# FanmingL/Recurrent-Offpolicy-RL

Hardware: AMD Instinct MI355X
Metric: env-steps/sec trained (higher is better)
Workload: dtype f32; 1 GPU; smamba_s32_c16_b2_nln SAC-REDQ update, B=64/GPU, T=1024, D=256 (configs[1]; N=8: configs[3]); row_length=1043, obs=17, act=6, critic=efc-8, global_rows=64, parallelism=dp1

## Files before the change

include/resel_hip.h:

```cpp
#ifndef RESEL_HIP_H
#define RESEL_HIP_H

#include <stddef.h>
#include <stdint.h>

#ifdef __cplusplus
extern "C" {
#endif

#define RESEL_OK 0
#define RESEL_EINVAL (-1)
#define RESEL_ELAUNCH (-2)

typedef void* resel_stream_t;

int resel_abi_version(void);
const char* resel_build_info(void);

enum {
    RESEL_PROF_SSCAN_FWD = 0, RESEL_PROF_SSCAN_BWD = 1, RESEL_PROF_ATTN_FWD = 2, RESEL_PROF_ATTN_DQ = 3, RESEL_PROF_ATTN_DKV = 4,
    RESEL_PROF_LINREC_REAL_FWD = 5, RESEL_PROF_LINREC_REAL_BWD = 6, RESEL_PROF_LINREC_COMPLEX_FWD = 7, RESEL_PROF_LINREC_COMPLEX_BWD = 8,
    RESEL_PROF_GRU_FWD = 9, RESEL_PROF_GRU_BWD = 10, RESEL_PROF_CONV_FWD = 11, RESEL_PROF_CONV_BWD = 12, RESEL_PROF_GEMM = 13,
    RESEL_PROF_SSCAN_FWD_LOCAL = 14, RESEL_PROF_SSCAN_BWD_LOCAL = 15,
    RESEL_PROF_NSLOTS = 16
};
int resel_profile_enable(int on);
int resel_profile_collect(int kernel_id, double* total_us, int* launches);

#define RESEL_SSCAN_CKPT 8
size_t resel_selective_scan_ckpt_bytes(int B, int L, int Di, int N);
size_t resel_selective_scan_fwd_workspace_bytes(int B, int L, int Di, int N, int time_segments);
int resel_selective_scan_fwd(const float* u, int64_t ld_u, const float* delta, int64_t ld_delta,
                             const float* z, int64_t ld_z, const float* A,
                             const float* Bm, int64_t ld_b, const float* Cm, int64_t ld_c,
                             const float* D, const float* delta_bias, const float* start,
                             float* out, int64_t ld_out, float* ckpt, float* last_state, void* workspace,
                             int B, int L, int Di, int N, int delta_softplus, int time_segments,
                             void* amax_out, unsigned amax_epoch, resel_stream_t stream);

size_t resel_selective_scan_bwd_workspace_bytes(int B, int L, int Di, int N, int time_segments);
int resel_selective_scan_bwd(const float* u, int64_t ld_u, const float* delta, int64_t ld_delta,
                             const float* z, int64_t ld_z, const float* A,
                             const float* Bm, int64_t ld_b, const float* Cm, int64_t ld_c,
                             const float* D, const float* delta_bias, const float* start,
                             const float* dout, int64_t ld_dout, const float* ckpt,
                             float* du, int64_t ld_du, float* ddelta, int64_t ld_ddelta, float* dz, int64_t ld_dz,
                             float* dBm, int64_t ld_db, float* dCm, int64_t ld_dc,
                             float* dA, float* dD, float* ddelta_bias, void* workspace,
                             int B, int L, int Di, int N, int delta_softplus, int time_segments,
                             void* amax_dz, void* amax_ddelta, unsigned amax_epoch, resel_stream_t stream);

int resel_causal_conv1d_fwd(const float* x, int64_t ld_x, const float* w, const float* bias, const float* mask,
                            float* y, int64_t ld_y, int B, int L, int Di, int K, int silu, void* amax_y, unsigned amax_epoch,
                            resel_stream_t stream);
size_t resel_causal_conv1d_bwd_workspace_bytes(int B, int L, int Di, int K);
int resel_causal_conv1d_bwd(const float* x, int64_t ld_x, const float* w, const float* bias, const float* mask,
                            const float* dy, int64_t ld_dy, float* dx, int64_t ld_dx, float* dw, float* dbias,
                            void* workspace, int B, int L, int Di, int K, int silu, void* amax_dx, unsigned amax_epoch,
                            resel_stream_t stream);
int resel_causal_conv1d_bwd2(const float* x, int64_t ld_x, const float* w, const float* bias, const float* mask,
                             const float* dy, int64_t ld_dy, const float* dy2, int64_t ld_dy2, float* dx, int64_t ld_dx,
                             float* dw, float* dbias, void* workspace, int B, int L, int Di, int K, int silu,
                             void* amax_dx, unsigned amax_epoch, resel_stream_t stream);

int resel_add_layernorm_fwd(const float* x, const float* residual, const float* w, const float* b,
                            float* y, float* res_out, float* stats, int M, int C, float eps, int rms, int act,
                            void* amax_y, unsigned amax_epoch, resel_stream_t stream);
size_t resel_add_layernorm_bwd_workspace_bytes(int M, int C);
int resel_add_layernorm_bwd(const float* dy, const float* dres_in, const float* res, const float* w, const float* b,
                            const float* stats, float* dx, float* dw, float* db, void* workspace,
                            int M, int C, int rms, int has_bias, int act, void* amax_dx, unsigned amax_epoch, resel_stream_t stream);

int resel_linrec_real_fwd(const float* v, const float* f, int64_t ld_u, const float* start, const float* h0, float* h,
                          int B, int L, int C, int fuse_act, void* amax_h, unsigned amax_epoch, resel_stream_t stream);
int resel_linrec_real_bwd(const float* v, const float* f, int64_t ld_u, const float* start, const float* h0, const float* h,
                          const float* dh, float* dv, float* df, int64_t ld_du, int B, int L, int C, int fuse_act,
                          void* amax_du, unsigned amax_epoch, resel_stream_t stream);
int resel_linrec_complex_fwd(const float* vr, const float* vi, int64_t ld_u, const float* lam_re, const float* lam_im,
                             const float* gamma, const float* start, const float* h0r, const float* h0i,
                             float* hr, float* hi, int B, int L, int C, void* amax_h, unsigned amax_epoch, resel_stream_t stream);
size_t resel_linrec_complex_bwd_workspace_bytes(int B, int L, int C);
int resel_linrec_complex_bwd(const float* vr, const float* vi, int64_t ld_u, const float* lam_re, const float* lam_im,
                             const float* gamma, const float* start, const float* h0r, const float* h0i,
                             const float* hr, const float* hi, const float* dhr, const float* dhi,
                             float* dvr, float* dvi, int64_t ld_du, float* dlam_re, float* dlam_im, float* dgamma,
                             void* workspace, int B, int L, int C, resel_stream_t stream);

int resel_lru_params_fwd(const float* params_log, float* out, int C, resel_stream_t stream);
int resel_lru_params_bwd(const float* params_log, const float* dout, float* dparams_log, int C, resel_stream_t stream);

size_t resel_gru_workspace_bytes(int B, int L, int H);
int resel_gru_seq_fwd(const float* gi, const float* w_hh, const float* b_hh, const float* h0,
                      float* h_all, float* gates, void* workspace, int B, int L, int H, resel_stream_t stream);
int resel_gru_seq_bwd(const float* w_hh, const float* h0, const float* h_all, const float* gates,
                      const float* dh_all, float* dgi, float* dgh, void* workspace,
                      int B, int L, int H, resel_stream_t stream);

size_t resel_gru_multi_workspace_bytes(int n_net, int B, int L, int H);
int resel_gru_multi_fwd(int n_net, const float* const* gi, const float* const* w_hh, const float* const* b_hh,
                        const float* const* h0, float* const* h_all, float* const* gates, void* workspace,
                        int B, int L, int H, resel_stream_t stream);
int resel_gru_multi_form(int n_net, int B, int H);

size_t resel_attn_varlen_fwd_workspace_bytes(int S, int max_seqlen);
int resel_attn_varlen_fwd(const uint16_t* qkv, const int32_t* cu_seqlens, const float* slopes, uint16_t* out, float* lse,
                          void* workspace, int T, int S, int H, int hd, int max_seqlen, float scale,
                          float p_drop, uint64_t seed, uint64_t offset, resel_stream_t stream);
size_t resel_attn_varlen_bwd_workspace_bytes(int T, int S, int H, int hd, int max_seqlen);
int resel_attn_varlen_bwd(const uint16_t* qkv, const int32_t* cu_seqlens, const float* slopes, const uint16_t* out,
                          const float* lse, const uint16_t* dout, uint16_t* dqkv, void* workspace,
                          int T, int S, int H, int hd, int max_seqlen, float scale,
                          float p_drop, uint64_t seed, uint64_t offset, resel_stream_t stream);

int resel_dropout(const float* x, float* y, int64_t n, float p_drop, uint64_t seed, uint64_t offset, resel_stream_t stream);
int resel_dropout_offset_base(const void* base);
int resel_gelu_dropout_fwd(const float* x, float* y, int64_t n, float p_drop, uint64_t seed, uint64_t offset,
                           void* amax_y, unsigned amax_epoch, resel_stream_t stream);
int resel_gelu_dropout_bwd(const float* x, const float* dy, float* dx, int64_t n, float p_drop, uint64_t seed, uint64_t offset,
                           void* amax_dx, unsigned amax_epoch, resel_stream_t stream);

int resel_tanh_gaussian_fwd(const float* out2, const float* noise, float* action_mean, float* action_sample,
                            float* logp, int M, int A, resel_stream_t stream);
int resel_tanh_gaussian_bwd(const float* out2, const float* noise, const float* d_sample, const float* d_logp,
                            float* d_out2, int M, int A, resel_stream_t stream);

int resel_sac_target(const float* q, const int32_t* subset, int m, const float* next_logp, const float* log_alpha,
                     const float* reward, const float* done, const float* mask, float gamma, float* guard,
                     float* target, float* stats, void* workspace, int E, int M, resel_stream_t stream);
int resel_sac_target_phase(int phase, const float* q, const int32_t* subset, int m, const float* next_logp, const float* log_alpha,
                           const float* reward, const float* done, const float* mask, float gamma, float* guard,
                           float* target, float* stats, float* extrema, void* workspace, int E, int M, resel_stream_t stream);
int resel_sac_target_local(const float* q, const int32_t* subset, int m, const float* next_logp, const float* log_alpha,
                           const float* reward, const float* done, const float* mask, float gamma, const float* guard,
                           float* target, float* stats, float* extrema, void* workspace, int E, int M, resel_stream_t stream);
int resel_guard_apply_slots(const float* slots, int world, float* guard, resel_stream_t stream);
size_t resel_sac_target_workspace_bytes(int M);

size_t resel_masked_loss_workspace_bytes(void);
int resel_q_loss_fwd(const float* q, const float* y, const float* mask, float* out2, void* workspace, int E, int M, resel_stream_t stream);
int resel_q_loss_bwd(const float* q, const float* y, const float* mask, const float* g, float* dq, int E, int M, resel_stream_t stream);
int resel_actor_loss_fwd(const float* logp, const float* q, const float* mask, const float* log_alpha, float* out2, void* workspace,
                         int E, int M, int use_logp, int reduce_min, resel_stream_t stream);
int resel_actor_loss_bwd(const float* q, const float* mask, const float* log_alpha, const float* g, float* dlogp, float* dq,
                         int E, int M, int use_logp, int reduce_min, resel_stream_t stream);

int resel_soft_update(float* target, const float* online, float tau, int64_t n, resel_stream_t stream);
int resel_adamw_flat(float* p, const float* g, float* m, float* v, int64_t n, const int64_t* seg_end,
                     const float* seg_lr, const float* seg_wd, int nseg, float beta1, float beta2, float eps,
                     int step, const float* grad_scale, resel_stream_t stream);
int resel_adamw_flat_bc(float* p, const float* g, float* m, float* v, int64_t n, const int64_t* seg_end,
                        const float* seg_lr, const float* seg_wd, int nseg, float beta1, float beta2, float eps,
                        float bc1, float bc2_sqrt, const float* grad_scale, resel_stream_t stream);
int resel_adamw_flat_dev(float* p, const float* g, float* m, float* v, int64_t n, const int64_t* seg_end,
                         const float* seg_lr, const float* seg_wd, int nseg, float beta1, float beta2, float eps,
                         const float* bias_corrections, const float* grad_scale, resel_stream_t stream);
size_t resel_sumsq_workspace_bytes(int64_t n);
int resel_sumsq(const float* x, int64_t n, float* out, void* workspace, resel_stream_t stream);

int resel_bias_act_fwd(float* y, const float* bias, int64_t rows, int C, int64_t rows_per_seg, int act, resel_stream_t stream);
size_t resel_bias_act_bwd_workspace_bytes(int64_t rows, int C, int64_t rows_per_seg);
int resel_bias_act_bwd(const float* g, int64_t ldg, const float* a, int64_t lda, float* gy, float* dbias, void* workspace, int64_t rows, int C,
                       int64_t rows_per_seg, int act, void* amax_gy, unsigned amax_epoch, resel_stream_t stream);

int resel_ensemble_head_fwd(float* y, const float* b2, const float* w3, const float* b3, float* q, int64_t rows, int H,
                            int64_t rows_per_seg, resel_stream_t stream);
size_t resel_ensemble_head_bwd_workspace_bytes(int64_t rows, int H, int64_t rows_per_seg);
int resel_ensemble_head_bwd(const float* gq, const float* a, const float* w3, float* gy, float* db2, float* dw3, void* workspace,
                            int64_t rows, int H, int64_t rows_per_seg, void* amax_gy, unsigned amax_epoch, resel_stream_t stream);

size_t resel_gemm_f32_workspace_bytes(int M, int N, int K, int batch);
int resel_gemm_f32(const float* A, int64_t lda, int64_t strideA, int a_kcontig,
                   const float* B, int64_t ldb, int64_t strideB, int b_kcontig,
                   const float* bias, int64_t strideBias, int act,
                   float* C, int64_t ldc, int64_t strideC, void* workspace,
                   int M, int N, int K, int batch, int split, resel_stream_t stream);

int resel_gemm_f32x(const float* A, int64_t lda, int64_t strideA, int a_kcontig,
                    const float* B, int64_t ldb, int64_t strideB, int b_kcontig,
                    const float* bias, int64_t strideBias, int act,
                    float* C, int64_t ldc, int64_t strideC, void* workspace,
                    int M, int N, int K, int batch, int split, const float* amax_a, const float* amax_b,
                    void* amax_c, unsigned amax_epoch, resel_stream_t stream);
int resel_gemm_f32_fused_supported(int kind, int M, int N, int K, int64_t lda, int64_t ldb);
size_t resel_gemm_f32_fused_workspace_bytes(int M, int N, int K, int batch, int kind);
int resel_gemm_f32_dact(const float* A, int64_t lda, int64_t strideA, int a_kcontig,
                        const float* B, int64_t ldb, int64_t strideB, int b_kcontig,
                        const float* Y, int64_t ldy, int64_t strideY,
                        float* C, int64_t ldc, int64_t strideC, float* dbias, void* workspace,
                        int M, int N, int K, int batch, const float* amax_a, const float* amax_b,
                        void* amax_c, unsigned amax_epoch, resel_stream_t stream);
int resel_gemm_f32_head(const float* A, int64_t lda, int64_t strideA, int a_kcontig,
                        const float* B, int64_t ldb, int64_t strideB, int b_kcontig,
                        const float* bias, int64_t strideBias, const float* w3, int64_t strideW3, const float* b3,
                        float* C, int64_t ldc, int64_t strideC, float* q, void* workspace,
                        int M, int N, int K, int batch, const float* amax_a, const float* amax_b,
                        void* amax_c, unsigned amax_epoch, resel_stream_t stream);
int resel_place_blocks(float* out, int64_t ld_out, int rows, int cols, int nblk, const float* const* src, const int64_t* ld_src,
                       const int* r0, const int* nr, const int* c0, const int* nc, resel_stream_t stream);

int resel_amax_segments(const float* flat, const int64_t* begin, const int64_t* len, int nseg, void* handles, unsigned epoch,
                        resel_stream_t stream);
size_t resel_amax_state_bytes(void);
int resel_amax(const float* x, int64_t ld, int64_t stride, int rows, int cols, int batch, void* out, unsigned epoch, void* state,
               resel_stream_t stream);
int resel_amax_check(const float* x, int64_t ld, int64_t stride, int rows, int cols, int batch, const void* handle, int* err, int tag,
                     resel_stream_t stream);

size_t resel_gemm_bf16_workspace_bytes(int M, int N, int K);
int resel_gemm_bf16(const void* A, int64_t lda, int a_kcontig, int a_bf16, const void* B, int64_t ldb, int b_kcontig, int b_bf16,
                    const float* bias, void* C, int64_t ldc, int c_bf16, void* workspace, int M, int N, int K,
                    resel_stream_t stream);

size_t resel_colsum_bf16_workspace_bytes(int M, int N);
int resel_colsum_bf16(const uint16_t* x, int64_t ld, int M, int N, float* out, void* workspace, resel_stream_t stream);

int resel_gather_trajs(const float* buffer, int W, int64_t capacity, const int* segments, int nseg, int max_len, int skip, int rows, int Tp,
                       int c_mask, int c_start, int c_done, int c_timeout, const int* pre_pairs, int npairs,
                       float* out, resel_stream_t stream);

int resel_mamba_conv_step(const float* x, int64_t ldx, const float* state_in, int64_t ld_in, float* state_out, int64_t ld_out,
                          int64_t stride_d, int64_t stride_k, int W, const float* w, const float* bias, float* xc, int B, int Di,
                          int K, int act, resel_stream_t stream);
int resel_selective_state_update(const float* state_in, int64_t ld_in, float* state_out, int64_t ld_out, const float* xc,
                                 const float* x_db, int64_t ld_xdb, const float* w_dt, const float* dt_bias, const float* A_log,
                                 const float* D, const float* z, int64_t ldz, float* y, int B, int Di, int N, int R,
                                 resel_stream_t stream);
int resel_attn_decode(const uint16_t* qkv, int64_t ld_qkv, uint16_t* kv_cache, const int32_t* pos_dev, int pos_host,
                      const float* slopes, uint16_t* out, float scale, int B, int H, int head_dim, int max_seqlen,
                      resel_stream_t stream);

size_t resel_atb_workspace_bytes(int64_t K, int Wd, int Nd);
int resel_atb(const float* wide, int64_t ldw, int Wd, const float* narrow, int64_t ldn, int Nd, float* out, int transposed,
              void* workspace, int64_t K, resel_stream_t stream);

#ifdef __cplusplus
}
#endif
#endif
```

recurrent-offpolicy-rl_amd/csrc/gemm_bf3.hip:

```cpp
#include "gemm_splitk.h"
#include <type_traits>

namespace {
using namespace resel;

typedef float f32x16 __attribute__((ext_vector_type(16)));
typedef __bf16 bf16x8 __attribute__((ext_vector_type(8)));
constexpr int BM = 256, BN = 128;
constexpr int NTH = 512;
constexpr int GRID = 256;
constexpr int TILE = BM * BN;
constexpr int ROWB = 64;
constexpr int PLA = BM * ROWB, PLB = BN * ROWB;
constexpr int STAGE = 3 * PLA + 3 * PLB;

struct Params {
    const float *A, *B, *bias;
    float *C, *slab;
    int64_t lda, ldb, ldc, sA, sB, sC, sBias;
    int M, N, K;
    int act;
    int mt, nt;
    int nfull, nsplit, nsl, kslice;
    const float *amaxA, *amaxB;
    AmaxOut amaxC;
    int ntst;
    const float* aux;
    int64_t ldaux, sAux;
    float* red;
    int redrows;
};

__device__ __forceinline__ int plane_off(int row, int c) {
    const int q = row >> 2;
    return ((row ^ (q & 1)) << 6) + ((c ^ (q & 3)) << 4);
}

__device__ __forceinline__ uint32_t rne_pair(float lo, float hi) {
    typedef __bf16 bf16x2_t __attribute__((ext_vector_type(2)));
    typedef float f32x2_t __attribute__((ext_vector_type(2)));
    const f32x2_t v = {lo, hi};
    return __builtin_bit_cast(uint32_t, __builtin_convertvector(v, bf16x2_t));
}
struct P3 { uint2 p1, p2, p3; };
template <int NP>
__device__ __forceinline__ P3 split4(const float4& v) {
#ifdef BF3_AB_NOSPLIT
    return P3{make_uint2(__float_as_uint(v.x), __float_as_uint(v.y)), make_uint2(__float_as_uint(v.z), __float_as_uint(v.w)),
              make_uint2(__float_as_uint(v.x), __float_as_uint(v.w))};
#endif
    const float x[4] = {v.x, v.y, v.z, v.w};
    uint32_t w1[2], w2[2], w3[2] = {0u, 0u};
#pragma unroll
    for (int q = 0; q < 2; ++q) {
        const uint32_t u0 = __float_as_uint(x[2 * q]), u1 = __float_as_uint(x[2 * q + 1]);
        w1[q] = __builtin_amdgcn_perm(u1, u0, 0x07060302u);
        const float r0 = x[2 * q] - __uint_as_float(u0 & 0xffff0000u), r1 = x[2 * q + 1] - __uint_as_float(u1 & 0xffff0000u);
        if (NP == 2) {
            w2[q] = rne_pair(r0, r1);
        } else {
            const uint32_t v0 = __float_as_uint(r0), v1 = __float_as_uint(r1);
            w2[q] = __builtin_amdgcn_perm(v1, v0, 0x07060302u);
            const float s0 = r0 - __uint_as_float(v0 & 0xffff0000u), s1 = r1 - __uint_as_float(v1 & 0xffff0000u);
            w3[q] = __builtin_amdgcn_perm(__float_as_uint(s1), __float_as_uint(s0), 0x07060302u);
        }
    }
    return P3{make_uint2(w1[0], w1[1]), make_uint2(w2[0], w2[1]), make_uint2(w3[0], w3[1])};
}
struct P3h { uint32_t p1, p2, p3; };
template <int NP>
__device__ __forceinline__ P3h split2(float x0, float x1) {
    const uint32_t u0 = __float_as_uint(x0), u1 = __float_as_uint(x1);
    P3h o;
    o.p1 = __builtin_amdgcn_perm(u1, u0, 0x07060302u);
    const float r0 = x0 - __uint_as_float(u0 & 0xffff0000u), r1 = x1 - __uint_as_float(u1 & 0xffff0000u);
    if (NP == 2) {
        o.p2 = rne_pair(r0, r1);
        o.p3 = 0u;
        return o;
    }
    const uint32_t v0 = __float_as_uint(r0), v1 = __float_as_uint(r1);
    o.p2 = __builtin_amdgcn_perm(v1, v0, 0x07060302u);
    const float s0 = r0 - __uint_as_float(v0 & 0xffff0000u), s1 = r1 - __uint_as_float(v1 & 0xffff0000u);
    o.p3 = __builtin_amdgcn_perm(__float_as_uint(s1), __float_as_uint(s0), 0x07060302u);
    return o;
}

typedef _Float16 f16x2_t __attribute__((ext_vector_type(2)));
typedef float f32x2_t __attribute__((ext_vector_type(2)));
template <bool WIDE>
__device__ __forceinline__ void split_pair_f16(float x0, float x1, f32x2_t sc, uint32_t& p1, uint32_t& p2, uint32_t& p3) {
#ifdef BF3_AB_NOSPLIT
    p1 = __float_as_uint(x0); p2 = __float_as_uint(x1); p3 = __float_as_uint(x0) ^ __float_as_uint(sc.x);
    return;
#endif
    const f32x2_t xs = {x0 * sc.x, x1 * sc.x};
    const f16x2_t h = __builtin_convertvector(xs, f16x2_t);
    p1 = __builtin_bit_cast(uint32_t, h);
    if (WIDE) {
        const f32x2_t r = {__builtin_fmaf((float)h.x, -2048.f, x0 * sc.y), __builtin_fmaf((float)h.y, -2048.f, x1 * sc.y)};
        p2 = __builtin_bit_cast(uint32_t, __builtin_convertvector(r, f16x2_t));
        p3 = 0u;
    } else {
        const f32x2_t r = {xs.x - (float)h.x, xs.y - (float)h.y};
        p2 = __builtin_bit_cast(uint32_t, __builtin_convertvector(r, f16x2_t));
        p3 = 0u;
    }
}
template <bool WIDE>
__device__ __forceinline__ P3 split4_f16(const float4& v, f32x2_t sc) {
    P3 o;
    split_pair_f16<WIDE>(v.x, v.y, sc, o.p1.x, o.p2.x, o.p3.x);
    split_pair_f16<WIDE>(v.z, v.w, sc, o.p1.y, o.p2.y, o.p3.y);
    return o;
}
template <bool WIDE>
__device__ __forceinline__ P3h split2_f16(float x0, float x1, f32x2_t sc) {
    P3h o;
    split_pair_f16<WIDE>(x0, x1, sc, o.p1, o.p2, o.p3);
    return o;
}
__device__ __forceinline__ float f16_scale(float amax) {
    const int f = (int)((__float_as_uint(amax) >> 23) & 0xffu);
    const int e = min(max(268 - f, 1), 240);
    return __uint_as_float((uint32_t)e << 23);
}

template <bool KC, int ROWS>
struct Src {
    static constexpr int NPC = ROWS / 64;
    static constexpr bool is_kc = KC;
    static constexpr int NR = KC ? NPC : (ROWS == 256 ? 4 : 2);
    const char* base;
    const char* base0;
    uint32_t off[NR];
    uint32_t loff[KC ? NPC : 4];
    int64_t step;
    int rl0, rlim, ld4, kofs4;
    int kofs;
    float4 r[NR];
    __device__ __forceinline__ void init(const float* P, int64_t ld, int rows, int r0, int k0, int tid) {
        if (KC) {
            kofs = 4 * (tid & 7);
            base = (const char*)(P + (int64_t)r0 * ld + k0);
            base0 = (const char*)(P + (int64_t)r0 * ld);
#pragma unroll
            for (int i = 0; i < NPC; ++i) {
                const int rl = (tid >> 3) + 64 * i;
                off[i] = (uint32_t)(((r0 + rl < rows ? rl : 0) * ld + kofs) * 4);
            }
            step = BK * 4;
            rl0 = tid >> 3;
            rlim = min(rows - 1 - r0, ROWS - 1);
            ld4 = (int)(ld * 4);
            kofs4 = kofs * 4;
        } else {
            const int g = ROWS == 256 ? (tid & 7) + 8 * (tid >> 6) : (tid & 7) + 8 * (tid >> 7);
            kofs = ROWS == 256 ? 4 * ((tid >> 3) & 7) : 2 * ((tid >> 3) & 15);
            base = (const char*)(P + (int64_t)k0 * ld + r0);
            base0 = (const char*)(P + r0);
            const int rl = 4 * g;
#pragma unroll
            for (int j = 0; j < NR; ++j) off[j] = (uint32_t)(((kofs + j) * ld + (r0 + rl < rows ? rl : 0)) * 4);
            step = (int64_t)BK * ld * 4;
        }
    }
    __device__ __forceinline__ void init_lds(int tid) {
        if (KC) {
#pragma unroll
            for (int i = 0; i < NPC; ++i) loff[i] = plane_off((tid >> 3) + 64 * i, (tid & 7) >> 1) + 8 * (tid & 1);
        } else if (ROWS == 256) {
            const int g = (tid & 7) + 8 * (tid >> 6), k4 = (tid >> 3) & 7;
#pragma unroll
            for (int j = 0; j < 4; ++j) loff[j] = plane_off(4 * g + j, k4 >> 1) + 8 * (k4 & 1);
        } else {
            const int g = (tid & 7) + 8 * (tid >> 7), k2 = (tid >> 3) & 15;
#pragma unroll
            for (int j = 0; j < 4; ++j) loff[j] = plane_off(4 * g + j, k2 >> 2) + 4 * (k2 & 3);
        }
    }
    __device__ __forceinline__ void load_sched(bool full) {
#ifdef BF3_AB_NOLOAD
        asm volatile("" : "+v"(r[0].x));
        return;
#endif
        const char* b = full ? base : base0;
#pragma unroll
        for (int i = 0; i < NR; ++i) r[i] = *reinterpret_cast<const float4*>(b + off[i]);
        if (full) base += step;
    }
    __device__ __forceinline__ void load(int k0, int kend) { load_to(r, k0, kend); }
    __device__ __forceinline__ void load_to(float4 (&r)[NR], int k0, int kend) {
#ifdef BF3_AB_NOLOAD
        asm volatile("" : "+v"(r[0].x));
        return;
#endif
        if (k0 + BK <= kend) {
#pragma unroll
            for (int i = 0; i < NR; ++i) r[i] = *reinterpret_cast<const float4*>(base + off[i]);
        } else {
#pragma unroll
            for (int i = 0; i < NR; ++i) {
                r[i] = make_float4(0.f, 0.f, 0.f, 0.f);
                if (k0 + kofs + (KC ? 0 : i) < kend) r[i] = *reinterpret_cast<const float4*>(base + off[i]);
            }
        }
        base += step;
    }
    __device__ __forceinline__ void load_piece(float4& v, int i, int k0, int kend) const {
#ifdef BF3_AB_NOLOAD
        asm volatile("" : "+v"(v.x));
        return;
#endif
        if (k0 + BK <= kend) {
            v = *reinterpret_cast<const float4*>(base + off[i]);
        } else {
            v = make_float4(0.f, 0.f, 0.f, 0.f);
            if (k0 + kofs + (KC ? 0 : i) < kend) v = *reinterpret_cast<const float4*>(base + off[i]);
        }
    }
    __device__ __forceinline__ void advance() { base += step; }
    __device__ __forceinline__ uint32_t piece_off(int i) const {
        return __umul24((uint32_t)min(rl0 + 64 * i, rlim), (uint32_t)ld4) + (uint32_t)kofs4;
    }
    template <int PL, int NP, int F16>
    __device__ __forceinline__ void store_piece(const float4& v, int i, char* pl, f32x2_t sc) const {
        static_assert(KC, "pieces exist in the [rows][K] layout only");
        const P3 s = F16 == 1 ? split4_f16<true>(v, sc) : F16 == 2 ? split4_f16<false>(v, sc) : split4<NP>(v);
        *reinterpret_cast<uint2*>(pl + loff[i]) = s.p1;
        *reinterpret_cast<uint2*>(pl + PL + loff[i]) = s.p2;
        if (NP == 3) *reinterpret_cast<uint2*>(pl + 2 * PL + loff[i]) = s.p3;
    }
    template <int PL, int NP, int F16 = 0>
    __device__ __forceinline__ void store(char* pl, f32x2_t sc = f32x2_t{1.f, 2048.f}) const { store_from<PL, NP, F16>(r, pl, sc); }
    template <int PL, int NP, int F16 = 0>
    __device__ __forceinline__ void store_from(const float4 (&r)[NR], char* pl, f32x2_t sc = f32x2_t{1.f, 2048.f}) const {
        if (KC) {
#pragma unroll
            for (int i = 0; i < NPC; ++i) {
                const P3 s = F16 == 1 ? split4_f16<true>(r[i], sc) : F16 == 2 ? split4_f16<false>(r[i], sc) : split4<NP>(r[i]);
                *reinterpret_cast<uint2*>(pl + loff[i]) = s.p1;
                *reinterpret_cast<uint2*>(pl + PL + loff[i]) = s.p2;
                if (NP == 3) *reinterpret_cast<uint2*>(pl + 2 * PL + loff[i]) = s.p3;
            }
        } else if (ROWS == 256) {
            const float c[4][4] = {{r[0].x, r[1].x, r[2].x, r[3].x}, {r[0].y, r[1].y, r[2].y, r[3].y},
                                   {r[0].z, r[1].z, r[2].z, r[3].z}, {r[0].w, r[1].w, r[2].w, r[3].w}};
#pragma unroll
            for (int j = 0; j < 4; ++j) {
                const float4 cj = make_float4(c[j][0], c[j][1], c[j][2], c[j][3]);
                const P3 s = F16 == 1 ? split4_f16<true>(cj, sc) : F16 == 2 ? split4_f16<false>(cj, sc) : split4<NP>(cj);
                *reinterpret_cast<uint2*>(pl + loff[j]) = s.p1;
                *reinterpret_cast<uint2*>(pl + PL + loff[j]) = s.p2;
                if (NP == 3) *reinterpret_cast<uint2*>(pl + 2 * PL + loff[j]) = s.p3;
            }
        } else {
            const float c[4][2] = {{r[0].x, r[1].x}, {r[0].y, r[1].y}, {r[0].z, r[1].z}, {r[0].w, r[1].w}};
#pragma unroll
            for (int j = 0; j < 4; ++j) {
                const P3h s = F16 == 1 ? split2_f16<true>(c[j][0], c[j][1], sc) : F16 == 2 ? split2_f16<false>(c[j][0], c[j][1], sc) : split2<NP>(c[j][0], c[j][1]);
                *reinterpret_cast<uint32_t*>(pl + loff[j]) = s.p1;
                *reinterpret_cast<uint32_t*>(pl + PL + loff[j]) = s.p2;
                if (NP == 3) *reinterpret_cast<uint32_t*>(pl + 2 * PL + loff[j]) = s.p3;
            }
        }
    }
};

struct Frag { bf16x8 a[3][2], b[3][2]; };

__device__ __forceinline__ bf16x8 lds16(const char* p) { return *reinterpret_cast<const bf16x8*>(p); }
template <int NP>
__device__ __forceinline__ void read_a(Frag& f, const char* fa) {
#pragma unroll
    for (int pi = 0; pi < NP; ++pi)
#pragma unroll
        for (int t = 0; t < 2; ++t) f.a[pi][t] = lds16(fa + pi * PLA + t * 32 * ROWB);
}
template <int NP>
__device__ __forceinline__ void read_b(Frag& f, const char* fb) {
#pragma unroll
    for (int pi = 0; pi < NP; ++pi)
#pragma unroll
        for (int t = 0; t < 2; ++t) f.b[pi][t] = lds16(fb + pi * PLB + t * 32 * ROWB);
}
typedef _Float16 f16x8 __attribute__((ext_vector_type(8)));
template <int P, int Q>
__device__ __forceinline__ void mfma_term_f16(f32x16 (&acc)[2][2], const Frag& f) {
#pragma unroll
    for (int a = 0; a < 2; ++a)
#pragma unroll
        for (int b = 0; b < 2; ++b) {
#ifdef BF3_AB_NOMFMA
            asm volatile("" :: "v"(f.a[P][a]), "v"(f.b[Q][b]));
#else
            acc[a][b] = __builtin_amdgcn_mfma_f32_32x32x16_f16(__builtin_bit_cast(f16x8, f.a[P][a]), __builtin_bit_cast(f16x8, f.b[Q][b]), acc[a][b], 0, 0, 0);
#endif
        }
}
template <int P, int Q>
__device__ __forceinline__ void mfma_term(f32x16 (&acc)[2][2], const Frag& f) {
#pragma unroll
    for (int a = 0; a < 2; ++a)
#pragma unroll
        for (int b = 0; b < 2; ++b) {
#ifdef BF3_AB_NOMFMA
            asm volatile("" :: "v"(f.a[P][a]), "v"(f.b[Q][b]));
#elif defined(BF3_AB_M16)
            {
                typedef float f32x4v __attribute__((ext_vector_type(4)));
                constexpr int h = ((P + Q) & 1) * 2;
                f32x4v q0 = __builtin_shufflevector(acc[a][b], acc[a][b], 4 * h, 4 * h + 1, 4 * h + 2, 4 * h + 3);
                f32x4v q1 = __builtin_shufflevector(acc[a][b], acc[a][b], 4 * h + 4, 4 * h + 5, 4 * h + 6, 4 * h + 7);
                q0 = __builtin_amdgcn_mfma_f32_16x16x32_bf16(f.a[P][a], f.b[Q][b], q0, 0, 0, 0);
                q1 = __builtin_amdgcn_mfma_f32_16x16x32_bf16(f.a[P][a], f.b[Q][b], q1, 0, 0, 0);
#pragma unroll
                for (int e = 0; e < 4; ++e) { acc[a][b][4 * h + e] = q0[e]; acc[a][b][4 * h + 4 + e] = q1[e]; }
            }
#else
            acc[a][b] = __builtin_amdgcn_mfma_f32_32x32x16_bf16(f.a[P][a], f.b[Q][b], acc[a][b], 0, 0, 0);
#endif
        }
}
template <int SPLIT>
__device__ __forceinline__ void mfma_small(f32x16 (&acc)[2][2], const Frag& f) {
    if (SPLIT == 3 || SPLIT == 2) return;
    mfma_term<2, 0>(acc, f); mfma_term<0, 2>(acc, f); mfma_term<1, 1>(acc, f);
}
__device__ __forceinline__ void mfma_lead(f32x16 (&acc)[2][2], const Frag& f) {
    mfma_term<1, 0>(acc, f); mfma_term<0, 1>(acc, f); mfma_term<0, 0>(acc, f);
}
__device__ __forceinline__ void mfma_lead_f16(f32x16 (&acc)[2][2], Frag& f) {
    const f16x8 k = {(_Float16)0.00048828125f, (_Float16)0.00048828125f, (_Float16)0.00048828125f, (_Float16)0.00048828125f,
// ... 336 lines not shown
                    if (MODE != 1) {
#pragma unroll
                        for (int i = 0; i < ST::NR; ++i) aload(regs[i], src.base, src.off[i]);
                    }
                }
            };
            using IA = std::integral_constant<int, PLA>;
            using IB = std::integral_constant<int, PLB>;
            one(a0, ra[S][0], st, scA, IA{}, std::true_type{});
            one(a1, ra[S][1], st, scA, IA{}, std::true_type{});
            one(b0, rb[S][0], st + 3 * PLA, scB, IB{}, std::false_type{});
            one(b1, rb[S][1], st + 3 * PLA, scB, IB{}, std::false_type{});
            if (MODE != 1) advance();
        };
        auto landed = [&]() {
#pragma unroll
            for (int q = 0; q < 2; ++q)
#pragma unroll
                for (int v = 0; v < 2; ++v) {
#pragma unroll
                    for (int i = 0; i < SA::NR; ++i) asm volatile("s_waitcnt vmcnt(0)" : "+v"(ra[q][v][i]) :: "memory");
#pragma unroll
                    for (int i = 0; i < SB::NR; ++i) asm volatile("s_waitcnt vmcnt(0)" : "+v"(rb[q][v][i]) :: "memory");
                }
        };
        using S0 = std::integral_constant<int, 0>;
        using S1 = std::integral_constant<int, 1>;
        using M0 = std::integral_constant<int, 0>;
        using M1 = std::integral_constant<int, 1>;
        using M2 = std::integral_constant<int, 2>;
        p_open();
        issue_set(S0{});
        if (nsteps > 1) issue_set(S1{});
        int j = 0;
        for (; j + 3 < nsteps; j += 2) {
            recycle(S0{}, M0{});
            WS_BARRIER();
            recycle(S1{}, M0{});
            WS_BARRIER();
        }
        landed();
        for (; j < nsteps; ++j) {
            const bool more = j + 2 < nsteps;
            if (j & 1) { if (more) recycle(S1{}, M2{}); else recycle(S1{}, M1{}); }
            else { if (more) recycle(S0{}, M2{}); else recycle(S0{}, M1{}); }
            if (more) landed();
            WS_BARRIER();
        }
        WS_BARRIER();
        return;
    }

    const float unscale = (1.f / sa_) * (1.f / sb_);
    const int lane = tid & 63, w = tid >> 6;
    const int wm = (w >> 1) * 128, wn = (w & 1) * 64;
    const int li = lane & 31, lh = lane >> 5;
    const char* fa[2];
    const char* fb[2];
#pragma unroll
    for (int s = 0; s < 2; ++s) {
        fa[s] = lds + wm * ROWB + plane_off(li, 2 * s + lh);
        fb[s] = lds + 3 * PLA + wn * ROWB + plane_off(li, 2 * s + lh);
    }
    struct F4 { f16x8 a[2][4], b[2][2]; };
    auto rd = [&](F4& f, const char* pa, const char* pb) {
#pragma unroll
        for (int pi = 0; pi < 2; ++pi) {
#pragma unroll
            for (int t = 0; t < 4; ++t) f.a[pi][t] = *reinterpret_cast<const f16x8*>(pa + pi * PLA + t * 32 * ROWB);
#pragma unroll
            for (int t = 0; t < 2; ++t) f.b[pi][t] = *reinterpret_cast<const f16x8*>(pb + pi * PLB + t * 32 * ROWB);
        }
    };
    f32x16 acc[4][2];
    auto mm = [&](const F4& f) {
        const f16x8 k = {(_Float16)0.00048828125f, (_Float16)0.00048828125f, (_Float16)0.00048828125f, (_Float16)0.00048828125f,
                         (_Float16)0.00048828125f, (_Float16)0.00048828125f, (_Float16)0.00048828125f, (_Float16)0.00048828125f};
        const f16x8 bs0 = f.b[0][0] * k, bs1 = f.b[0][1] * k;
#ifdef BF3_AB_NOMFMA
#pragma unroll
        for (int a = 0; a < 4; ++a) asm volatile("" :: "v"(f.a[0][a]), "v"(f.a[1][a]), "v"(bs0), "v"(bs1), "v"(f.b[0][0]), "v"(f.b[0][1]), "v"(f.b[1][0]), "v"(f.b[1][1]));
        return;
#endif
#pragma unroll
        for (int a = 0; a < 4; ++a) {
            acc[a][0] = __builtin_amdgcn_mfma_f32_32x32x16_f16(f.a[1][a], bs0, acc[a][0], 0, 0, 0);
            acc[a][1] = __builtin_amdgcn_mfma_f32_32x32x16_f16(f.a[1][a], bs1, acc[a][1], 0, 0, 0);
        }
#pragma unroll
        for (int q = 1; q >= 0; --q)
#pragma unroll
            for (int a = 0; a < 4; ++a) {
                acc[a][0] = __builtin_amdgcn_mfma_f32_32x32x16_f16(f.a[0][a], f.b[q][0], acc[a][0], 0, 0, 0);
                acc[a][1] = __builtin_amdgcn_mfma_f32_32x32x16_f16(f.a[0][a], f.b[q][1], acc[a][1], 0, 0, 0);
            }
    };
    float cmax = 0.f;
    F4 f0, f1;
    WS_BARRIER();
    rd(f0, fa[0], fb[0]);
    int cur_st = 0;
    constexpr bool DEFER_F0 = EPI == 4;
    for (int c_item = blockIdx.x; c_item < total; c_item += G) {
        const Item cur = decode<BM, BN>(p, c_item);
        if (DEFER_F0 && c_item != (int)blockIdx.x) rd(f0, fa[0] + cur_st * STAGE, fb[0] + cur_st * STAGE);
        float zero = 0.f;
        asm volatile("" : "+v"(zero));
#pragma unroll
        for (int a = 0; a < 4; ++a)
#pragma unroll
            for (int b = 0; b < 2; ++b)
#pragma unroll
                for (int e = 0; e < 16; ++e) acc[a][b][e] = zero;
        float bv[2] = {0.f, 0.f};
        for (int c_k0 = cur.kbeg; c_k0 < cur.kend; c_k0 += BK) {
            const int so = cur_st * STAGE, sn = (cur_st ^ 1) * STAGE;
            if (c_k0 + BK >= cur.kend && p.bias && !cur.split) {
#pragma unroll
                for (int b = 0; b < 2; ++b) {
                    const int n = cur.n0 + wn + 32 * b + li;
                    bv[b] = p.bias[(int64_t)cur.z * p.sBias + (n < p.N ? n : 0)];
                }
            }
            BF3_FENCE();
            rd(f1, fa[1] + so, fb[1] + so);
            mm(f0);
#pragma unroll
            for (int i = 0; i < 12; ++i) {
                __builtin_amdgcn_sched_group_barrier(0x008, 1, 0);
                __builtin_amdgcn_sched_group_barrier(0x100, 1, 0);
            }
            BF3_FENCE();
            WS_BARRIER();
            BF3_FENCE();
            if (!(DEFER_F0 && c_k0 + BK >= cur.kend)) rd(f0, fa[0] + sn, fb[0] + sn);
            mm(f1);
#pragma unroll
            for (int i = 0; i < 12; ++i) {
                __builtin_amdgcn_sched_group_barrier(0x008, 1, 0);
                __builtin_amdgcn_sched_group_barrier(0x100, 1, 0);
            }
            BF3_FENCE();
            cur_st ^= 1;
        }
#ifdef BF3_AB_NOEPI
        if (lane == 0) p.C[(int64_t)cur.m0 * p.ldc + cur.n0 + w] = acc[0][0][0] + acc[1][1][1] + acc[2][0][2] + acc[3][1][3];
        continue;
#endif
#pragma unroll
        for (int a = 0; a < 4; ++a)
#pragma unroll
            for (int b = 0; b < 2; ++b)
#pragma unroll
                for (int e = 0; e < 16; ++e) acc[a][b][e] *= unscale;
        if (cur.split) {
            float* o = p.slab + (int64_t)(cur.split - 1) * TILE + (wm + 4 * lh) * BN + wn + li;
#pragma unroll
            for (int a = 0; a < 4; ++a)
#pragma unroll
                for (int b = 0; b < 2; ++b)
#pragma unroll
                    for (int e = 0; e < 16; ++e) o[(32 * a + (e & 3) + 8 * (e >> 2)) * BN + 32 * b] = acc[a][b][e];
            continue;
        }
        if constexpr (EPI == 0) {
            float* C = p.C + (int64_t)cur.z * p.sC;
            const bool full_m = cur.m0 + BM <= p.M;
            if (full_m && cur.n0 + BN <= p.N && p.act != 2) {
                char* sc = lds + (w >> 1) * STAGE + 2 * PLA + (w & 1) * 5120;
                float* wr = reinterpret_cast<float*>(sc) + (4 * lh) * 40 + li;
                const float4* rdp = reinterpret_cast<const float4*>(sc + (lane >> 3) * 160 + (lane & 7) * 16);
#pragma unroll
                for (int b = 0; b < 2; ++b) {
#pragma unroll
                    for (int a = 0; a < 4; ++a) {
                        float v[16];
#pragma unroll
                        for (int e = 0; e < 16; ++e) v[e] = acc[a][b][e] + bv[b];
                        if (p.act == 1) {
#pragma unroll
                            for (int e = 0; e < 16; ++e) v[e] = elu1(v[e]);
                        }
                        if (p.act == 3) {
#pragma unroll
                            for (int e = 0; e < 16; ++e) v[e] = softplus_nb(v[e]);
                        }
                        if (p.amaxC.slot) {
#pragma unroll
                            for (int e = 0; e < 16; e += 2) cmax = fmaxf(cmax, fmaxf(__builtin_fabsf(v[e]), __builtin_fabsf(v[e + 1])));
                        }
#pragma unroll
                        for (int e = 0; e < 16; ++e) wr[((e & 3) + 8 * (e >> 2)) * 40] = v[e];
                        float* q = C + (int64_t)(cur.m0 + wm + 32 * a + (lane >> 3)) * p.ldc + cur.n0 + wn + 32 * b + 4 * (lane & 7);
#pragma unroll
                        for (int g = 0; g < 4; ++g) {
                            const float4 t = rdp[g * 8 * 10];
                            if (p.ntst) {
                                typedef float f4v __attribute__((ext_vector_type(4)));
                                __builtin_nontemporal_store(f4v{t.x, t.y, t.z, t.w}, reinterpret_cast<f4v*>(q + (int64_t)(8 * g) * p.ldc));
                            } else {
                                *reinterpret_cast<float4*>(q + (int64_t)(8 * g) * p.ldc) = t;
                            }
                        }
                    }
                }
                continue;
            }
#pragma unroll
            for (int b = 0; b < 2; ++b) {
                const int n = cur.n0 + wn + 32 * b + li;
                if (n >= p.N) continue;
#pragma unroll
                for (int a = 0; a < 4; ++a) {
                    float v[16];
#pragma unroll
                    for (int e = 0; e < 16; ++e) v[e] = acc[a][b][e] + bv[b];
                    if (p.act == 1) {
#pragma unroll
                        for (int e = 0; e < 16; ++e) v[e] = elu1(v[e]);
                    }
                    if (p.act == 3) {
#pragma unroll
                        for (int e = 0; e < 16; ++e) v[e] = softplus_nb(v[e]);
                    }
                    const int mb = cur.m0 + wm + 32 * a + 4 * lh;
                    float* crow = C + (int64_t)mb * p.ldc + n;
                    if (p.act == 2) {
#pragma unroll
                        for (int e = 0; e < 16; ++e) {
                            const int dm = (e & 3) + 8 * (e >> 2);
                            if (mb + dm < p.M) v[e] += crow[(int64_t)dm * p.ldc];
                        }
                    }
                    if (full_m) {
#pragma unroll
                        for (int e = 0; e < 16; ++e) crow[(int64_t)((e & 3) + 8 * (e >> 2)) * p.ldc] = v[e];
                    } else {
#pragma unroll
                        for (int e = 0; e < 16; ++e) {
                            const int dm = (e & 3) + 8 * (e >> 2);
                            if (mb + dm < p.M) crow[(int64_t)dm * p.ldc] = v[e];
                        }
                    }
                    if (p.amaxC.slot) {
#pragma unroll
                        for (int e = 0; e < 16; e += 2) cmax = fmaxf(cmax, fmaxf(__builtin_fabsf(v[e]), __builtin_fabsf(v[e + 1])));
                    }
                }
            }
        } else {
            float* C = p.C + (int64_t)cur.z * p.sC;
            const bool full_m = cur.m0 + BM <= p.M;
            constexpr bool DACT = EPI == 4, HEAD = EPI == 5;
            const int act = EPI ? (HEAD ? 1 : 0) : p.act;
            if constexpr (DACT) {
                constexpr int PF = 3;
                const int lane = (int)__builtin_amdgcn_mbcnt_hi(~0u, __builtin_amdgcn_mbcnt_lo(~0u, 0u));
                const int li = lane & 31, lh = lane >> 5;
                const int w = __builtin_amdgcn_readfirstlane(threadIdx.x >> 6);
                const int wm = (w >> 1) * 128, wn = (w & 1) * 64;
                typedef float f32x4a __attribute__((ext_vector_type(4)));
                f32x4a yv[8][4];
                char* sc = lds + (w >> 1) * STAGE + 2 * PLA + (w & 1) * 5120;
                float* wr = reinterpret_cast<float*>(sc) + (4 * lh) * 40 + li;
                float4* rdp = reinterpret_cast<float4*>(sc + (lane >> 3) * 160 + (lane & 7) * 16);
                const uint32_t ylane = (uint32_t)(((lane >> 3) * (int)p.ldaux + 4 * (lane & 7)) * 4);
                const float* ybase = p.aux + (int64_t)cur.z * p.sAux + (int64_t)(cur.m0 + wm) * p.ldaux + cur.n0 + wn;
                auto yld = [](f32x4a& r, uint32_t off, const float* base) {
                    asm volatile("global_load_dwordx4 %0, %1, %2" : "=v"(r) : "v"(off), "s"(base) : "memory");
                };
                auto ywait = [](f32x4a& r0, f32x4a& r1, f32x4a& r2, f32x4a& r3, auto NC) {
                    asm volatile("s_waitcnt vmcnt(%4)" : "+v"(r0), "+v"(r1), "+v"(r2), "+v"(r3) : "n"(decltype(NC)::value) : "memory");
                };
                auto yload = [&](auto TC) {
                    constexpr int t = decltype(TC)::value;
                    if constexpr (t < 8) {
                        const float* yb = ybase + (int64_t)(32 * (t >> 1)) * p.ldaux + 32 * (t & 1);
#pragma unroll
                        for (int g = 0; g < 4; ++g) yld(yv[t][g], ylane, yb + (int64_t)(8 * g) * p.ldaux);
                    }
                };
                float cs[2] = {0.f, 0.f}, cmx = 0.f;
                auto mul = [&](auto TC) {
                    constexpr int t = decltype(TC)::value;
                    constexpr int a = t >> 1, b = t & 1;
                    yload(std::integral_constant<int, t + PF>{});
                    ywait(yv[t][0], yv[t][1], yv[t][2], yv[t][3], std::integral_constant<int, 4 * ((t + PF < 7 ? t + PF : 7) - t)>{});
#pragma unroll
                    for (int g = 0; g < 4; ++g) rdp[g * 8 * 10] = make_float4(yv[t][g].x, yv[t][g].y, yv[t][g].z, yv[t][g].w);
#pragma unroll
                    for (int e = 0; e < 16; ++e) {
                        const float y = wr[((e & 3) + 8 * (e >> 2)) * 40];
                        const float v = acc[a][b][e] * (y > 0.f ? 1.f : y + 1.f);
                        acc[a][b][e] = v;
                        cs[b] += v;
                        cmx = fmaxf(cmx, __builtin_fabsf(v));
                    }
                };
                yload(std::integral_constant<int, 0>{}); yload(std::integral_constant<int, 1>{}); yload(std::integral_constant<int, 2>{});
                static_assert(PF == 3, "the prologue issues PF tiles");
                mul(std::integral_constant<int, 0>{}); mul(std::integral_constant<int, 1>{}); mul(std::integral_constant<int, 2>{});
                mul(std::integral_constant<int, 3>{}); mul(std::integral_constant<int, 4>{}); mul(std::integral_constant<int, 5>{});
                mul(std::integral_constant<int, 6>{}); mul(std::integral_constant<int, 7>{});
                if (p.red) {
#pragma unroll
                    for (int b = 0; b < 2; ++b) {
                        const float c = cs[b] + __shfl_xor(cs[b], 32, 64);
                        if (lh == 0) p.red[((int64_t)cur.z * p.redrows + 2 * (cur.m0 / BM) + (w >> 1)) * p.N + cur.n0 + wn + 32 * b + li] = c;
                    }
                }
                amax_publish_wave(cmx, p.amaxC);
#pragma unroll
                for (int b = 0; b < 2; ++b) {
#pragma unroll
                    for (int a = 0; a < 4; ++a) {
#pragma unroll
                        for (int e = 0; e < 16; ++e) wr[((e & 3) + 8 * (e >> 2)) * 40] = acc[a][b][e];
                        float* q = C + (int64_t)(cur.m0 + wm + 32 * a + (lane >> 3)) * p.ldc + cur.n0 + wn + 32 * b + 4 * (lane & 7);
#pragma unroll
                        for (int g = 0; g < 4; ++g) {
                            const float4 t = rdp[g * 8 * 10];
                            typedef float f4v __attribute__((ext_vector_type(4)));
                            __builtin_nontemporal_store(f4v{t.x, t.y, t.z, t.w}, reinterpret_cast<f4v*>(q + (int64_t)(8 * g) * p.ldc));
                        }
                    }
                }
                continue;
            }
            if (full_m && cur.n0 + BN <= p.N && act != 2) {
                char* sc = lds + (w >> 1) * STAGE + 2 * PLA + (w & 1) * 5120;
                float* wr = reinterpret_cast<float*>(sc) + (4 * lh) * 40 + li;
                const float4* rdp = reinterpret_cast<const float4*>(sc + (lane >> 3) * 160 + (lane & 7) * 16);
                auto tile = [&](int a, int b, const float4 (&yv)[4], float4& cs, const float4& w3, float (&qr)[4]) {
                    float v[16];
#pragma unroll
                    for (int e = 0; e < 16; ++e) v[e] = acc[a][b][e] + bv[b];
                    if (act == 1) {
#pragma unroll
                        for (int e = 0; e < 16; ++e) v[e] = elu1(v[e]);
                    }
                    if (act == 3) {
#pragma unroll
                        for (int e = 0; e < 16; ++e) v[e] = softplus_nb(v[e]);
                    }
                    if (p.amaxC.slot && !DACT) {
#pragma unroll
                        for (int e = 0; e < 16; e += 2) cmax = fmaxf(cmax, fmaxf(__builtin_fabsf(v[e]), __builtin_fabsf(v[e + 1])));
                    }
#pragma unroll
                    for (int e = 0; e < 16; ++e) wr[((e & 3) + 8 * (e >> 2)) * 40] = v[e];
                    float* q = C + (int64_t)(cur.m0 + wm + 32 * a + (lane >> 3)) * p.ldc + cur.n0 + wn + 32 * b + 4 * (lane & 7);
#pragma unroll
                    for (int g = 0; g < 4; ++g) {
                        float4 t = rdp[g * 8 * 10];
                        if (DACT) {
                            t.x *= yv[g].x > 0.f ? 1.f : yv[g].x + 1.f; t.y *= yv[g].y > 0.f ? 1.f : yv[g].y + 1.f;
                            t.z *= yv[g].z > 0.f ? 1.f : yv[g].z + 1.f; t.w *= yv[g].w > 0.f ? 1.f : yv[g].w + 1.f;
                            cs.x += t.x; cs.y += t.y; cs.z += t.z; cs.w += t.w;
                            if (p.amaxC.slot) cmax = amax4(cmax, t);
                        }
                        if (HEAD) qr[g] += (t.x * w3.x + t.y * w3.y) + (t.z * w3.z + t.w * w3.w);
                        if (p.ntst) {
                            typedef float f4v __attribute__((ext_vector_type(4)));
                            __builtin_nontemporal_store(f4v{t.x, t.y, t.z, t.w}, reinterpret_cast<f4v*>(q + (int64_t)(8 * g) * p.ldc));
                        } else {
                            *reinterpret_cast<float4*>(q + (int64_t)(8 * g) * p.ldc) = t;
                        }
                    }
                };
                if constexpr (EPI == 0) {
                    const float4 z4 = make_float4(0.f, 0.f, 0.f, 0.f);
                    const float4 nov[4] = {z4, z4, z4, z4};
                    float4 ncs = z4;
                    float nq[4] = {0.f, 0.f, 0.f, 0.f};
#pragma unroll
                    for (int b = 0; b < 2; ++b)
#pragma unroll
                        for (int a = 0; a < 4; ++a) tile(a, b, nov, ncs, z4, nq);
                } else {
                    const float4 z4 = make_float4(0.f, 0.f, 0.f, 0.f);
                    {
                        const float4 nov[4] = {z4, z4, z4, z4};
                        float4 ncs = z4, w3[2];
#pragma unroll
                        for (int b = 0; b < 2; ++b) w3[b] = ld4(p.aux + (int64_t)cur.z * p.sAux + cur.n0 + wn + 32 * b + 4 * (lane & 7));
#pragma unroll
                        for (int a = 0; a < 4; ++a) {
                            float qr[4] = {0.f, 0.f, 0.f, 0.f};
#pragma unroll
                            for (int b = 0; b < 2; ++b) tile(a, b, nov, ncs, w3[b], qr);
                            float* qp = p.red + ((int64_t)cur.z * 2 * p.nt + 2 * (cur.n0 / BN) + (w & 1)) * p.M + cur.m0 + wm + 32 * a + (lane >> 3);
#pragma unroll
                            for (int g = 0; g < 4; ++g) {
                                float r = qr[g];
                                r += __shfl_xor(r, 1, 64); r += __shfl_xor(r, 2, 64); r += __shfl_xor(r, 4, 64);
                                if ((lane & 7) == 0) qp[8 * g] = r;
                            }
                        }
                    }
                }
                continue;
            }
            float cs1[2] = {0.f, 0.f};
#pragma unroll
            for (int a = 0; a < 4; ++a) {
                float qe[16];
                if (HEAD) {
#pragma unroll
                    for (int e = 0; e < 16; ++e) qe[e] = 0.f;
                }
                const int mb = cur.m0 + wm + 32 * a + 4 * lh;
#pragma unroll
                for (int b = 0; b < 2; ++b) {
                    const int n = cur.n0 + wn + 32 * b + li;
                    if (n >= p.N) continue;
                    float v[16];
#pragma unroll
                    for (int e = 0; e < 16; ++e) v[e] = acc[a][b][e] + bv[b];
                    if (act == 1) {
#pragma unroll
                        for (int e = 0; e < 16; ++e) v[e] = elu1(v[e]);
                    }
                    if (act == 3) {
#pragma unroll
                        for (int e = 0; e < 16; ++e) v[e] = softplus_nb(v[e]);
                    }
                    if (DACT) {
                        const float* yrow = p.aux + (int64_t)cur.z * p.sAux + (int64_t)mb * p.ldaux + n;
#pragma unroll
                        for (int e = 0; e < 16; ++e) {
                            const int dm = (e & 3) + 8 * (e >> 2);
                            float y = 0.f;
                            if (mb + dm < p.M) y = yrow[(int64_t)dm * p.ldaux]; else v[e] = 0.f;
                            v[e] *= y > 0.f ? 1.f : y + 1.f;
                            cs1[b] += v[e];
                        }
                    }
                    if (HEAD) {
                        const float w3 = p.aux[(int64_t)cur.z * p.sAux + n];
#pragma unroll
                        for (int e = 0; e < 16; ++e) qe[e] += v[e] * w3;
                    }
                    float* crow = C + (int64_t)mb * p.ldc + n;
                    if (act == 2) {
#pragma unroll
                        for (int e = 0; e < 16; ++e) {
                            const int dm = (e & 3) + 8 * (e >> 2);
                            if (mb + dm < p.M) v[e] += crow[(int64_t)dm * p.ldc];
                        }
                    }
                    if (full_m) {
#pragma unroll
                        for (int e = 0; e < 16; ++e) crow[(int64_t)((e & 3) + 8 * (e >> 2)) * p.ldc] = v[e];
                    } else {
#pragma unroll
                        for (int e = 0; e < 16; ++e) {
                            const int dm = (e & 3) + 8 * (e >> 2);
                            if (mb + dm < p.M) crow[(int64_t)dm * p.ldc] = v[e];
                        }
                    }
                    if (p.amaxC.slot) {
#pragma unroll
                        for (int e = 0; e < 16; e += 2) cmax = fmaxf(cmax, fmaxf(__builtin_fabsf(v[e]), __builtin_fabsf(v[e + 1])));
                    }
                }
                if (HEAD) {
                    float* qp = p.red + ((int64_t)cur.z * 2 * p.nt + 2 * (cur.n0 / BN) + (w & 1)) * p.M;
#pragma unroll
                    for (int e = 0; e < 16; ++e) {
                        float r = qe[e];
#pragma unroll
                        for (int o = 1; o < 32; o <<= 1) r += __shfl_xor(r, o, 64);
                        const int m = mb + (e & 3) + 8 * (e >> 2);
                        if (li == 0 && m < p.M) qp[m] = r;
                    }
                }
            }
            if (DACT && p.red) {
#pragma unroll
                for (int b = 0; b < 2; ++b) {
                    const int n = cur.n0 + wn + 32 * b + li;
                    const float c = cs1[b] + __shfl_xor(cs1[b], 32, 64);
                    if (lh == 0 && n < p.N) p.red[((int64_t)cur.z * 2 * p.mt + 2 * (cur.m0 / BM) + (w >> 1)) * p.N + n] = c;
                }
            }
        }
    }
    amax_publish_wave(cmax, p.amaxC);
}

template <bool AKC, bool BKC, int SP>
int launch_one(const Params& p, dim3 grid, hipStream_t s) {
    static std::atomic<bool> attr_set[64];
    return launch_big_lds(gemm_bf3_kernel<AKC, BKC, SP>, attr_set, grid, dim3(NTH), 2 * STAGE, s, p);
}
template <bool AKC, bool BKC, int EPI = 0>
int launch_ws(const Params& p, dim3 grid, hipStream_t s) {
    static std::atomic<bool> attr_set[64];
    return launch_big_lds(gemm_ws_kernel<AKC, BKC, EPI>, attr_set, grid, dim3(NTH_WS), WS_LDS, s, p);
}

constexpr int g_nt = 1;

}

#ifdef BF3_AB_CLOCK
extern "C" int resel_bf3_debug_clock(unsigned long long* host_out) {
    return (int)hipMemcpyFromSymbol(host_out, HIP_SYMBOL(g_bf3_clock), sizeof(unsigned long long) * 2 * GRID);
}
#endif

namespace resel {

size_t gemm_bf3_workspace_bytes(int M, int N, int K, int batch) {
    const Plan pl = make_plan<BM, BN, GRID>(M, N, K, batch);
    return (size_t)pl.nsplit * pl.nsl * TILE * sizeof(float);
}

bool gemm_bf3_fused_ok(int M, int N, int K, int64_t lda, int64_t ldb) {
    return M > 128 && N >= 4 && K >= BK && K % BK == 0 && lda < (1 << 22) && ldb < (1 << 22);
}

int gemm_bf3_launch(const float* A, int64_t lda, int64_t strideA, int a_kcontig, const float* B, int64_t ldb, int64_t strideB, int b_kcontig,
                    const float* bias, int64_t strideBias, int act, float* C, int64_t ldc, int64_t strideC, void* workspace,
                    int M, int N, int K, int batch, int split, hipStream_t s, const float* amaxA, const float* amaxB,
                    unsigned long long* amax_c, unsigned amax_epoch, const float* aux, int64_t ldaux, int64_t strideAux, float* red, int redrows) {
    if (split == 2 && (!amaxA || !amaxB)) return RESEL_EINVAL;
    Plan pl = make_plan<BM, BN, GRID>(M, N, K, batch);
    if (act >= 4) {
        if (split != 2 || !gemm_bf3_fused_ok(M, N, K, lda, ldb) || !aux) return RESEL_EINVAL;
        if (act == 4 && (M % BM || N % BN)) return RESEL_EINVAL;
        const long nbt = (long)((M + BM - 1) / BM) * ((N + BN - 1) / BN) * batch;
        pl = Plan{(int)nbt, 0, 1, (K + BK - 1) / BK * BK};
    }
    if (pl.nsplit && (!workspace || !aligned16(workspace))) return RESEL_EINVAL;
    Params p{A, B, bias, C, (float*)workspace, lda, ldb, ldc, strideA, strideB, strideC, strideBias, M, N, K, act,
             (M + BM - 1) / BM, (N + BN - 1) / BN, pl.nfull, pl.nsplit, pl.nsl, pl.kslice, amaxA, amaxB, AmaxOut{amax_c, amax_epoch}, g_nt,
             aux, ldaux, strideAux, red, redrows};
    const int64_t total = (int64_t)pl.nfull + (int64_t)pl.nsplit * pl.nsl;
    dim3 grid((unsigned)std::min<int64_t>(total, GRID));
    int rc;
#define BF3_LAUNCH(SP) \
    do { if (a_kcontig && b_kcontig) rc = launch_one<true, true, SP>(p, grid, s); \
         else if (a_kcontig) rc = launch_one<true, false, SP>(p, grid, s); \
         else if (b_kcontig) rc = launch_one<false, true, SP>(p, grid, s); \
         else rc = launch_one<false, false, SP>(p, grid, s); } while (0)
    const bool ws = split == 2 && K % BK == 0 && pl.kslice % BK == 0 && lda < (1 << 22) && ldb < (1 << 22);
    if (act >= 4) {
        if (!a_kcontig) return RESEL_EINVAL;
        if (act == 4) rc = b_kcontig ? launch_ws<true, true, 4>(p, grid, s) : launch_ws<true, false, 4>(p, grid, s);
        else rc = b_kcontig ? launch_ws<true, true, 5>(p, grid, s) : launch_ws<true, false, 5>(p, grid, s);
    } else if (ws) {
        if (a_kcontig && b_kcontig) rc = launch_ws<true, true>(p, grid, s);
        else if (a_kcontig) rc = launch_ws<true, false>(p, grid, s);
        else if (b_kcontig) rc = launch_ws<false, true>(p, grid, s);
        else rc = launch_ws<false, false>(p, grid, s);
    } else if (split == 3) BF3_LAUNCH(3); else if (split == 2) BF3_LAUNCH(2); else BF3_LAUNCH(6);
#undef BF3_LAUNCH
    if (rc != RESEL_OK) return rc;
    if (pl.nsplit) hipLaunchKernelGGL((gemm_fixup_kernel<BM, BN, Params>), dim3(TILE / 4 / 64, pl.nsplit), dim3(64, 4), 0, s, p);
#ifdef BF3_AB_FIXUP2
    if (pl.nsplit && act != 2) hipLaunchKernelGGL((gemm_fixup_kernel<BM, BN, Params>), dim3(TILE / 4 / 64, pl.nsplit), dim3(64, 4), 0, s, p);
#endif
    return launch_status();
}

}
```

recurrent-offpolicy-rl_amd/csrc/gemm_f32.hip:

```cpp
#include "gemm_splitk.h"

namespace resel {
size_t gemm_bf3_workspace_bytes(int M, int N, int K, int batch);
int gemm_bf3_launch(const float* A, int64_t lda, int64_t strideA, int a_kcontig, const float* B, int64_t ldb, int64_t strideB, int b_kcontig,
                    const float* bias, int64_t strideBias, int act, float* C, int64_t ldc, int64_t strideC, void* workspace,
                    int M, int N, int K, int batch, int split, hipStream_t s, const float* amaxA, const float* amaxB,
                    unsigned long long* amax_c, unsigned amax_epoch, const float* aux = nullptr, int64_t ldaux = 0, int64_t strideAux = 0,
                    float* red = nullptr, int redrows = 0);
bool gemm_bf3_fused_ok(int M, int N, int K, int64_t lda, int64_t ldb);
}

namespace {
using namespace resel;

typedef float f32x16 __attribute__((ext_vector_type(16)));
constexpr int BM = 128, BN = 128, NG = BK / 8;
constexpr int LDK = BK + 4;
constexpr int GRID = 512;
constexpr int TILE = BM * BN;

struct GemmParams {
    const float *A, *B, *bias;
    float *C, *slab;
    int64_t lda, ldb, ldc, sA, sB, sC, sBias;
    int M, N, K;
    int act;
    int mt, nt;
    int nfull;
    int nsplit, nsl, kslice;
    AmaxOut amaxC;
};

template <bool KC>
struct Src {
    const char* base;
    const char* base0;
    uint32_t off[4];
    int64_t step;
    int kofs;
    __device__ __forceinline__ void init(const float* P, int64_t ld, int rows, int r0, int k0, int tid) {
        kofs = 4 * (tid & 7);
        if (KC) {
            base = (const char*)(P + (int64_t)r0 * ld + k0);
            base0 = (const char*)(P + (int64_t)r0 * ld);
#pragma unroll
            for (int i = 0; i < 4; ++i) {
                const int rl = (tid >> 3) + 32 * i;
                off[i] = (uint32_t)(((r0 + rl < rows ? rl : 0) * ld + kofs) * 4);
            }
            step = BK * 4;
        } else {
            base = (const char*)(P + (int64_t)k0 * ld + r0);
            base0 = (const char*)(P + r0);
            const int rl = 4 * (tid >> 3);
#pragma unroll
            for (int j = 0; j < 4; ++j) off[j] = (uint32_t)(((kofs + j) * ld + (r0 + rl < rows ? rl : 0)) * 4);
            step = (int64_t)BK * ld * 4;
        }
    }
    __device__ __forceinline__ void load_sched(float4 (&r)[4], bool full) {
        const char* b = full ? base : base0;
#pragma unroll
        for (int i = 0; i < 4; ++i) r[i] = *reinterpret_cast<const float4*>(b + off[i]);
        if (full) base += step;
    }
    __device__ __forceinline__ void load(float4 (&r)[4], int k0, int kend) {
        if (k0 + BK <= kend) {
#pragma unroll
            for (int i = 0; i < 4; ++i) r[i] = *reinterpret_cast<const float4*>(base + off[i]);
        } else {
#pragma unroll
            for (int i = 0; i < 4; ++i) {
                r[i] = make_float4(0.f, 0.f, 0.f, 0.f);
                if (k0 + kofs + (KC ? 0 : i) < kend) r[i] = *reinterpret_cast<const float4*>(base + off[i]);
            }
        }
        base += step;
    }
};
template <bool KC>
__device__ __forceinline__ void tile_store(float* __restrict__ S, int tid, const float4 (&r)[4]) {
    if (KC) {
#pragma unroll
        for (int i = 0; i < 4; ++i) st4(S + ((tid >> 3) + 32 * i) * LDK + 4 * (tid & 7), r[i]);
    } else {
        float* q = S + (4 * (tid >> 3)) * LDK + 4 * (tid & 7);
        st4(q, make_float4(r[0].x, r[1].x, r[2].x, r[3].x));
        st4(q + LDK, make_float4(r[0].y, r[1].y, r[2].y, r[3].y));
        st4(q + 2 * LDK, make_float4(r[0].z, r[1].z, r[2].z, r[3].z));
        st4(q + 3 * LDK, make_float4(r[0].w, r[1].w, r[2].w, r[3].w));
    }
}

struct Frags { float4 a[NG][2], b[NG][2]; };
struct Planes;
template <int SPLIT>
__device__ __forceinline__ void read_frags(Frags& f, const float* __restrict__ As, const float* __restrict__ Bs, int g) {
    const int ko = SPLIT ? 16 * (g >> 1) + 4 * (g & 1) : 8 * g;
#pragma unroll
    for (int t = 0; t < 2; ++t) {
        f.a[g][t] = ld4(As + 32 * t * LDK + ko);
        f.b[g][t] = ld4(Bs + 32 * t * LDK + ko);
    }
}
__device__ __forceinline__ void read_a(Frags& f, const float* __restrict__ As, int g) {
#pragma unroll
    for (int t = 0; t < 2; ++t) f.a[g][t] = ld4(As + 32 * t * LDK + 16 * (g >> 1) + 4 * (g & 1));
}
__device__ __forceinline__ void read_b(Frags& f, const float* __restrict__ Bs, int g) {
#pragma unroll
    for (int t = 0; t < 2; ++t) f.b[g][t] = ld4(Bs + 32 * t * LDK + 16 * (g >> 1) + 4 * (g & 1));
}
template <int SPLIT>
__device__ __forceinline__ void quarter(f32x16 (&acc)[2][2], const Frags& f, Planes (&pl)[2], int q);
__device__ __forceinline__ void mfma_group(f32x16 (&acc)[2][2], const Frags& f, int g) {
#pragma unroll
    for (int a = 0; a < 2; ++a)
#pragma unroll
        for (int b = 0; b < 2; ++b) {
            acc[a][b] = __builtin_amdgcn_mfma_f32_32x32x2f32(f.a[g][a].x, f.b[g][b].x, acc[a][b], 0, 0, 0);
            acc[a][b] = __builtin_amdgcn_mfma_f32_32x32x2f32(f.a[g][a].y, f.b[g][b].y, acc[a][b], 0, 0, 0);
            acc[a][b] = __builtin_amdgcn_mfma_f32_32x32x2f32(f.a[g][a].z, f.b[g][b].z, acc[a][b], 0, 0, 0);
            acc[a][b] = __builtin_amdgcn_mfma_f32_32x32x2f32(f.a[g][a].w, f.b[g][b].w, acc[a][b], 0, 0, 0);
        }
}
typedef __bf16 bf16x8 __attribute__((ext_vector_type(8)));
struct Planes { bf16x8 a[3][2], b[3][2]; };

__device__ __forceinline__ void split8(const float4& lo, const float4& hi, bf16x8& p1, bf16x8& p2, bf16x8& p3) {
#ifdef GEMM_AB_NOSPLIT
    p1 = __builtin_bit_cast(bf16x8, lo); p2 = __builtin_bit_cast(bf16x8, hi); p3 = p1;
    return;
#endif
    const float x[8] = {lo.x, lo.y, lo.z, lo.w, hi.x, hi.y, hi.z, hi.w};
    uint32_t w1[4], w2[4], w3[4];
#pragma unroll
    for (int q = 0; q < 4; ++q) {
        const uint32_t u0 = __float_as_uint(x[2 * q]), u1 = __float_as_uint(x[2 * q + 1]);
        w1[q] = __builtin_amdgcn_perm(u1, u0, 0x07060302u);
        const float r0 = x[2 * q] - __uint_as_float(u0 & 0xffff0000u), r1 = x[2 * q + 1] - __uint_as_float(u1 & 0xffff0000u);
        const uint32_t v0 = __float_as_uint(r0), v1 = __float_as_uint(r1);
        w2[q] = __builtin_amdgcn_perm(v1, v0, 0x07060302u);
        const float s0 = r0 - __uint_as_float(v0 & 0xffff0000u), s1 = r1 - __uint_as_float(v1 & 0xffff0000u);
        w3[q] = __builtin_amdgcn_perm(__float_as_uint(s1), __float_as_uint(s0), 0x07060302u);
    }
    p1 = __builtin_bit_cast(bf16x8, make_uint4(w1[0], w1[1], w1[2], w1[3]));
    p2 = __builtin_bit_cast(bf16x8, make_uint4(w2[0], w2[1], w2[2], w2[3]));
    p3 = __builtin_bit_cast(bf16x8, make_uint4(w3[0], w3[1], w3[2], w3[3]));
}
__device__ __forceinline__ void split_a(Planes& pl, const Frags& f, int s) {
#pragma unroll
    for (int t = 0; t < 2; ++t) split8(f.a[2 * s][t], f.a[2 * s + 1][t], pl.a[0][t], pl.a[1][t], pl.a[2][t]);
}
__device__ __forceinline__ void split_b(Planes& pl, const Frags& f, int s) {
#pragma unroll
    for (int t = 0; t < 2; ++t) split8(f.b[2 * s][t], f.b[2 * s + 1][t], pl.b[0][t], pl.b[1][t], pl.b[2][t]);
}
template <int NM, int NV, int MEM = 0>
__device__ __forceinline__ void interleave_mfma_valu() {
#pragma unroll
    for (int i = 0; i < NM; ++i) {
        __builtin_amdgcn_sched_group_barrier(0x008, 1, 0);
        __builtin_amdgcn_sched_group_barrier(0x002, NV, 0);
        if (MEM == 2 && i < 8) __builtin_amdgcn_sched_group_barrier(0x200, 1, 0);
        if (MEM == 2 && i < 8) __builtin_amdgcn_sched_group_barrier(0x020, 1, 0);
        if (MEM != 0 && i >= 8) __builtin_amdgcn_sched_group_barrier(0x100, 1, 0);
    }
}
template <int P, int Q>
__device__ __forceinline__ void mfma_term(f32x16 (&acc)[2][2], const Planes& pl) {
#pragma unroll
    for (int a = 0; a < 2; ++a)
#pragma unroll
        for (int b = 0; b < 2; ++b) {
#ifdef GEMM_AB_NOMFMA
            asm volatile("" :: "v"(pl.a[P][a]), "v"(pl.b[Q][b]));
#else
            acc[a][b] = __builtin_amdgcn_mfma_f32_32x32x16_bf16(pl.a[P][a], pl.b[Q][b], acc[a][b], 0, 0, 0);
#endif
        }
}
template <int SPLIT>
__device__ __forceinline__ void mfma_terms(f32x16 (&acc)[2][2], const Planes& pl, int half) {
    if (half == 0) {
        mfma_term<2, 0>(acc, pl); mfma_term<0, 2>(acc, pl); mfma_term<1, 1>(acc, pl);
    } else {
        mfma_term<1, 0>(acc, pl); mfma_term<0, 1>(acc, pl); mfma_term<0, 0>(acc, pl);
    }
}

template <int SPLIT>
__device__ __forceinline__ void quarter(f32x16 (&acc)[2][2], const Frags& f, Planes (&pl)[2], int q) {
    mfma_group(acc, f, q);
}
template <int SPLIT, int Q, int MEM>
__device__ __forceinline__ void split_quarter(f32x16 (&acc)[2][2], const Frags& f, Planes (&pl)[2]) {
    if (Q == 0) split_b(pl[1], f, 1);
    if (Q == 1) split_a(pl[1], f, 1);
    if (Q == 2) split_a(pl[0], f, 0);
    if (Q == 3) split_b(pl[0], f, 0);
    mfma_terms<SPLIT>(acc, pl[Q >> 1], Q & 1);
    Planes& np = pl[Q < 2 ? 1 : 0];
#pragma unroll
    for (int pi = 0; pi < 3; ++pi)
#pragma unroll
        for (int t = 0; t < 2; ++t) {
            if (Q == 0 || Q == 3) asm volatile("" : "+v"(np.b[pi][t]));
            else asm volatile("" : "+v"(np.a[pi][t]));
        }
    interleave_mfma_valu<12, 8, MEM>();
}

#define RESEL_FENCE() __builtin_amdgcn_sched_barrier(0)
#ifdef GEMM_STAMP
__device__ unsigned long long g_gemm_stamps[64 * 16];
#define STAMP(i) do { if (stamp_on && stamp_step < 64) g_gemm_stamps[stamp_step * 16 + (i)] = __builtin_amdgcn_s_memtime(); } while (0)
#else
#define STAMP(i) do { } while (0)
#endif

template <bool AKC, bool BKC, int SPLIT>
__global__ __launch_bounds__(256, 2) void gemm_f32_kernel(GemmParams p) {
    constexpr int ASZ = BM * LDK, BSZ = BN * LDK;
    __shared__ __attribute__((aligned(16))) float lds[2 * (ASZ + BSZ)];
    const int tid = threadIdx.x, lane = tid & 63, w = tid >> 6;
    const int wm = (w >> 1) * 64, wn = (w & 1) * 64;
    const int li = lane & 31, lh = lane >> 5;
    const int total = p.nfull + p.nsplit * p.nsl;
    const int G = gridDim.x;
    if ((int)blockIdx.x >= total) return;

    Src<AKC> sa;
    Src<BKC> sb;
    float4 ra[4], rb[4];
    int p_item = blockIdx.x, p_k0, p_kend;
    bool p_live = true;
    auto p_open = [&]() {
        const Item it = decode<BM, BN>(p, p_item);
        sa.init(p.A + (int64_t)it.z * p.sA, p.lda, p.M, it.m0, it.kbeg, tid);
        sb.init(p.B + (int64_t)it.z * p.sB, p.ldb, p.N, it.n0, it.kbeg, tid);
        p_k0 = it.kbeg; p_kend = it.kend;
    };
    auto produce = [&]() {
        if (!p_live) return;
        sa.load(ra, p_k0, p_kend);
        sb.load(rb, p_k0, p_kend);
        p_k0 += BK;
        if (p_k0 >= p_kend) {
            p_item += G;
            if (p_item < total) p_open(); else p_live = false;
        }
    };
    int c_item = blockIdx.x;
    float* const lA = lds + (wm + li) * LDK + (SPLIT ? 8 : 4) * lh;
    float* const lB = lds + ASZ + (wn + li) * LDK + (SPLIT ? 8 : 4) * lh;
    Frags f;
    Planes pl[2];
    p_open();
    produce();
    tile_store<AKC>(lds, tid, ra);
    tile_store<BKC>(lds + ASZ, tid, rb);
    produce();
    if (SPLIT) {
        tile_store<AKC>(lds + ASZ + BSZ, tid, ra);
        tile_store<BKC>(lds + ASZ + BSZ + ASZ, tid, rb);
        produce();
    }
    __syncthreads();
#pragma unroll
    for (int g = 0; g < NG; ++g) read_frags<SPLIT>(f, lA, lB, g);
    if (SPLIT) { split_a(pl[0], f, 0); split_b(pl[0], f, 0); }
    int nb = ASZ + BSZ;
    float cmax = 0.f;
#ifdef GEMM_STAMP
    const bool stamp_on = blockIdx.x == 0 && tid == 0;
    int stamp_step = 0;
#endif
    for (; c_item < total; c_item += G) {
        const Item cur = decode<BM, BN>(p, c_item);
        float zero = 0.f;
        asm volatile("" : "+v"(zero));
        f32x16 acc[2][2];
#pragma unroll
        for (int a = 0; a < 2; ++a)
#pragma unroll
            for (int b = 0; b < 2; ++b)
#pragma unroll
                for (int e = 0; e < 16; ++e) acc[a][b][e] = zero;
        float bv[2] = {0.f, 0.f};
        for (int c_k0 = cur.kbeg; c_k0 < cur.kend; c_k0 += BK) {
            if (SPLIT) {
                const int cb = ASZ + BSZ - nb;
                RESEL_FENCE();
                STAMP(0);
                read_a(f, lA + cb, 2); read_a(f, lA + cb, 3);
                split_quarter<SPLIT, 0, 3>(acc, f, pl);
                RESEL_FENCE();
                STAMP(1);
                __syncthreads();
                STAMP(2);
                if (c_k0 + BK >= cur.kend && p.bias && !cur.split) {
#pragma unroll
                    for (int b = 0; b < 2; ++b) {
                        const int n = cur.n0 + wn + 32 * b + li;
                        bv[b] = p.bias[(int64_t)cur.z * p.sBias + (n < p.N ? n : 0)];
                    }
                }
                const float* nA = lA + nb;
                const float* nB = lB + nb;
                const bool fast = p_live && p_k0 + BK <= p_kend;
                RESEL_FENCE();
                tile_store<AKC>(lds + cb, tid, ra);
                tile_store<BKC>(lds + cb + ASZ, tid, rb);
                sa.load_sched(ra, fast);
                sb.load_sched(rb, fast);
                read_a(f, nA, 0); read_a(f, nA, 1);
                split_quarter<SPLIT, 1, 2>(acc, f, pl);
                RESEL_FENCE();
                if (fast) {
                    p_k0 += BK;
                    if (p_k0 >= p_kend) {
                        p_item += G;
                        if (p_item < total) p_open(); else p_live = false;
                    }
                } else {
                    produce();
                }
                RESEL_FENCE();
                STAMP(3);
                read_b(f, nB, 0); read_b(f, nB, 1);
                split_quarter<SPLIT, 2, 3>(acc, f, pl);
                RESEL_FENCE();
                STAMP(4);
                read_b(f, nB, 2); read_b(f, nB, 3);
                split_quarter<SPLIT, 3, 3>(acc, f, pl);
                RESEL_FENCE();
                STAMP(5);
#ifdef GEMM_STAMP
                ++stamp_step;
#endif
            } else {
                RESEL_FENCE();
                quarter<SPLIT>(acc, f, pl, 0);
                RESEL_FENCE();
                tile_store<AKC>(lds + nb, tid, ra);
                tile_store<BKC>(lds + nb + ASZ, tid, rb);
                RESEL_FENCE();
                quarter<SPLIT>(acc, f, pl, 1);
                RESEL_FENCE();
                if (c_k0 + BK >= cur.kend && p.bias && !cur.split) {
#pragma unroll
                    for (int b = 0; b < 2; ++b) {
                        const int n = cur.n0 + wn + 32 * b + li;
                        bv[b] = p.bias[(int64_t)cur.z * p.sBias + (n < p.N ? n : 0)];
                    }
                }
                produce();
                RESEL_FENCE();
                quarter<SPLIT>(acc, f, pl, 2);
                RESEL_FENCE();
                __syncthreads();
                read_frags<SPLIT>(f, lA + nb, lB + nb, 0);
                read_frags<SPLIT>(f, lA + nb, lB + nb, 1);
                read_frags<SPLIT>(f, lA + nb, lB + nb, 2);
                RESEL_FENCE();
                quarter<SPLIT>(acc, f, pl, 3);
                RESEL_FENCE();
                read_frags<SPLIT>(f, lA + nb, lB + nb, 3);
                RESEL_FENCE();
            }
            nb = ASZ + BSZ - nb;
        }
        if (cur.split) {
            float* o = p.slab + (int64_t)(cur.split - 1) * TILE + (wm + 4 * lh) * BN + wn + li;
#pragma unroll
            for (int a = 0; a < 2; ++a)
#pragma unroll
                for (int b = 0; b < 2; ++b)
#pragma unroll
                    for (int e = 0; e < 16; ++e) o[(32 * a + (e & 3) + 8 * (e >> 2)) * BN + 32 * b] = acc[a][b][e];
        } else {
            float* C = p.C + (int64_t)cur.z * p.sC;
            const bool full_m = cur.m0 + BM <= p.M;
#pragma unroll
            for (int b = 0; b < 2; ++b) {
                const int n = cur.n0 + wn + 32 * b + li;
                if (n >= p.N) continue;
#pragma unroll
                for (int a = 0; a < 2; ++a) {
                    float v[16];
#pragma unroll
                    for (int e = 0; e < 16; ++e) v[e] = acc[a][b][e] + bv[b];
                    if (p.act == 1) {
#pragma unroll
                        for (int e = 0; e < 16; ++e) v[e] = elu1(v[e]);
                    }
                    if (p.act == 3) {
#pragma unroll
                        for (int e = 0; e < 16; ++e) v[e] = softplus_nb(v[e]);
                    }
                    const int mb = cur.m0 + wm + 32 * a + 4 * lh;
                    float* crow = C + (int64_t)mb * p.ldc + n;
                    if (p.act == 2) {
#pragma unroll
                        for (int e = 0; e < 16; ++e) {
                            const int dm = (e & 3) + 8 * (e >> 2);
                            if (mb + dm < p.M) v[e] += crow[(int64_t)dm * p.ldc];
                        }
                    }
                    if (full_m) {
#pragma unroll
                        for (int e = 0; e < 16; ++e) crow[(int64_t)((e & 3) + 8 * (e >> 2)) * p.ldc] = v[e];
                    } else {
#pragma unroll
                        for (int e = 0; e < 16; ++e) {
                            const int dm = (e & 3) + 8 * (e >> 2);
                            if (mb + dm < p.M) crow[(int64_t)dm * p.ldc] = v[e];
                        }
                    }
                    if (p.amaxC.slot) {
#pragma unroll
                        for (int e = 0; e < 16; e += 2) cmax = fmaxf(cmax, fmaxf(__builtin_fabsf(v[e]), __builtin_fabsf(v[e + 1])));
                    }
                }
            }
        }
    }
    amax_publish_wave(cmax, p.amaxC);
}

}

#ifdef GEMM_STAMP
extern "C" int resel_gemm_debug_stamps(unsigned long long* host_out) {
    return (int)hipMemcpyFromSymbol(host_out, HIP_SYMBOL(g_gemm_stamps), sizeof(unsigned long long) * 64 * 16);
}
#endif

extern "C" size_t resel_gemm_f32_workspace_bytes(int M, int N, int K, int batch) {
    if (M <= 0 || N <= 0 || K <= 0 || batch <= 0) return 0;
    const Plan pl = make_plan<BM, BN, GRID>(M, N, K, batch);
    return std::max(std::max((size_t)pl.nsplit * pl.nsl * TILE * sizeof(float), gemm_bf3_workspace_bytes(M, N, K, batch)),
                    gemm_any_workspace_bytes(M, N, K, batch));
}

extern "C" int resel_gemm_f32(const float* A, int64_t lda, int64_t strideA, int a_kcontig,
                              const float* B, int64_t ldb, int64_t strideB, int b_kcontig,
                              const float* bias, int64_t strideBias, int act,
                              float* C, int64_t ldc, int64_t strideC, void* workspace,
                              int M, int N, int K, int batch, int split, resel_stream_t stream) {
    if (split == 2) return RESEL_EINVAL;
    return resel_gemm_f32x(A, lda, strideA, a_kcontig, B, ldb, strideB, b_kcontig, bias, strideBias, act, C, ldc, strideC, workspace,
                           M, N, K, batch, split, nullptr, nullptr, nullptr, 0u, stream);
}

extern "C" int resel_gemm_f32x(const float* A, int64_t lda, int64_t strideA, int a_kcontig,
                               const float* B, int64_t ldb, int64_t strideB, int b_kcontig,
                               const float* bias, int64_t strideBias, int act,
                               float* C, int64_t ldc, int64_t strideC, void* workspace,
                               int M, int N, int K, int batch, int split, const float* amax_a, const float* amax_b,
                               void* amax_c, unsigned amax_epoch, resel_stream_t stream) {
    if (!A || !B || !C || M <= 0 || N <= 0 || K <= 0 || batch <= 0 || act < 0 || act > 3) return RESEL_EINVAL;
    if (split != 0 && split != 2 && split != 3 && split != 6) return RESEL_EINVAL;
    if (split == 2 && (!amax_a || !amax_b)) return RESEL_EINVAL;
    if (amax_c && (reinterpret_cast<uintptr_t>(amax_c) & 7u)) return RESEL_EINVAL;
    if (split == 2 && M <= 128) split = 6;
    if (K < BK) split = 0;
    if (lda <= 0 || ldb <= 0 || ldc <= 0) return RESEL_EINVAL;
    const bool mfma_ok = !(lda % 4 || ldb % 4 || strideA % 4 || strideB % 4 || !aligned16(A) || !aligned16(B) || (a_kcontig ? K : M) % 4 ||
                           (b_kcontig ? K : N) % 4 || lda >= (int64_t)1 << 22 || ldb >= (int64_t)1 << 22);
    if (!mfma_ok || gemm_any_rows_ok(A, lda, strideA, a_kcontig, 0, B, ldb, strideB, b_kcontig, M, K, act))
        return gemm_any_launch(A, lda, strideA, a_kcontig, B, ldb, strideB, b_kcontig, bias, strideBias, act, C, ldc, strideC, workspace, M, N, K,
                               batch, 0, (unsigned long long*)amax_c, amax_epoch, (hipStream_t)stream);
    if ((split == 2 || split == 3 || split == 6) && M > 128)
        return gemm_bf3_launch(A, lda, strideA, a_kcontig, B, ldb, strideB, b_kcontig, bias, strideBias, act, C, ldc, strideC, workspace,
                               M, N, K, batch, split, (hipStream_t)stream, amax_a, amax_b, (unsigned long long*)amax_c, amax_epoch);
    if (split == 3) split = 6;
    const Plan pl = make_plan<BM, BN, GRID>(M, N, K, batch);
    if (pl.nsplit && (!workspace || !aligned16(workspace))) return RESEL_EINVAL;
    GemmParams p{A, B, bias, C, (float*)workspace, lda, ldb, ldc, strideA, strideB, strideC, strideBias, M, N, K, act,
                 (M + BM - 1) / BM, (N + BN - 1) / BN, pl.nfull, pl.nsplit, pl.nsl, pl.kslice, AmaxOut{(unsigned long long*)amax_c, amax_epoch}};
    const int64_t total = (int64_t)pl.nfull + (int64_t)pl.nsplit * pl.nsl;
    dim3 grid((unsigned)std::min<int64_t>(total, GRID));
    hipStream_t s = (hipStream_t)stream;
#define RESEL_GEMM_LAUNCH(SP) \
    do { if (a_kcontig && b_kcontig) launch_timed(RESEL_PROF_GEMM, gemm_f32_kernel<true, true, SP>, grid, dim3(256), 0, s, p); \
         else if (a_kcontig) launch_timed(RESEL_PROF_GEMM, gemm_f32_kernel<true, false, SP>, grid, dim3(256), 0, s, p); \
         else if (b_kcontig) launch_timed(RESEL_PROF_GEMM, gemm_f32_kernel<false, true, SP>, grid, dim3(256), 0, s, p); \
         else launch_timed(RESEL_PROF_GEMM, gemm_f32_kernel<false, false, SP>, grid, dim3(256), 0, s, p); } while (0)
    if (split == 6) RESEL_GEMM_LAUNCH(6);
    else RESEL_GEMM_LAUNCH(0);
#undef RESEL_GEMM_LAUNCH
    if (pl.nsplit) hipLaunchKernelGGL((gemm_fixup_kernel<BM, BN, GemmParams>), dim3(TILE / 4 / 64, pl.nsplit), dim3(64, 4), 0, s, p);
    return launch_status();
}

namespace {
__global__ __launch_bounds__(256) void head_fold_kernel(const float* __restrict__ part, int parts, int M, const float* __restrict__ b3, float* __restrict__ q) {
    const int z = blockIdx.y;
    const int m = blockIdx.x * 256 + threadIdx.x;
    if (m >= M) return;
    const float* pz = part + (int64_t)z * parts * M + m;
    float acc = b3 ? b3[z] : 0.f;
    for (int j = 0; j < parts; ++j) acc += pz[(int64_t)j * M];
    q[(int64_t)z * M + m] = acc;
}
bool fused_args_ok(const float* A, int64_t lda, int64_t strideA, int a_kcontig, const float* B, int64_t ldb, int64_t strideB, int b_kcontig,
                   const float* C, int64_t ldc, int M, int N, int K, int batch, const float* amax_a, const float* amax_b, const void* amax_c,
                   const void* workspace) {
    if (!A || !B || !C || M <= 0 || N <= 0 || K <= 0 || batch <= 0 || !amax_a || !amax_b || !workspace || !aligned16(workspace)) return false;
    if (amax_c && (reinterpret_cast<uintptr_t>(amax_c) & 7u)) return false;
    if (lda % 4 || ldb % 4 || ldc % 4 || strideA % 4 || strideB % 4 || !aligned16(A) || !aligned16(B) || !aligned16(C)) return false;
    if ((a_kcontig ? K : M) % 4 || (b_kcontig ? K : N) % 4 || N % 4) return false;
    if (lda <= 0 || ldb <= 0 || ldc <= 0) return false;
    return gemm_bf3_fused_ok(M, N, K, lda, ldb);
}
}

extern "C" int resel_gemm_f32_fused_supported(int kind, int M, int N, int K, int64_t lda, int64_t ldb) {
    if (kind == 4) return (M >= 256 && N % 128 == 0 && gemm_bf3_fused_ok(M, N, K, lda, ldb)) ? 1 : 0;
    if (kind == 5) return gemm_bf3_fused_ok(M, N, K, lda, ldb) ? 1 : 0;
    return 0;
}

extern "C" size_t resel_gemm_f32_fused_workspace_bytes(int M, int N, int K, int batch, int kind) {
    if (M <= 0 || N <= 0 || K <= 0 || batch <= 0) return 0;
    const size_t mt = M / 256, nt = (N + 127) / 128;
    const size_t own = (kind == 5 ? 2 * nt * (size_t)M : (2 * mt + 1) * (size_t)N) * batch * sizeof(float);
    return own + (kind == 4 && M % 256 ? resel_gemm_f32_workspace_bytes(M % 256, N, K, batch) + 256 : 0);
}

namespace {
__global__ __launch_bounds__(256) void dact_tail_kernel(float* __restrict__ C, int64_t ldc, int64_t sC, const float* __restrict__ Y, int64_t ldy, int64_t sY,
                                                        int rows, int N, float* __restrict__ part, int64_t part_stride, AmaxOut amax) {
    __shared__ float s_sum[4][64];
    const int c = blockIdx.x * 64 + (threadIdx.x & 63), rg = threadIdx.x >> 6, z = blockIdx.y;
    float acc = 0.f, mx = 0.f;
    if (c < N) {
        float* Cz = C + (int64_t)z * sC + c;
        const float* Yz = Y + (int64_t)z * sY + c;
        for (int r = rg; r < rows; r += 4) {
            const float y = Yz[(int64_t)r * ldy];
            const float v = Cz[(int64_t)r * ldc] * (y > 0.f ? 1.f : y + 1.f);
            Cz[(int64_t)r * ldc] = v;
            acc += v;
            mx = fmaxf(mx, __builtin_fabsf(v));
        }
    }
    s_sum[rg][threadIdx.x & 63] = acc;
    __syncthreads();
    if (rg == 0 && c < N && part) part[(int64_t)z * part_stride + c] = (s_sum[0][threadIdx.x] + s_sum[1][threadIdx.x]) + (s_sum[2][threadIdx.x] + s_sum[3][threadIdx.x]);
    amax_publish_wave(mx, amax);
}
}

extern "C" int resel_gemm_f32_dact(const float* A, int64_t lda, int64_t strideA, int a_kcontig,
                                   const float* B, int64_t ldb, int64_t strideB, int b_kcontig,
                                   const float* Y, int64_t ldy, int64_t strideY,
                                   float* C, int64_t ldc, int64_t strideC, float* dbias, void* workspace,
                                   int M, int N, int K, int batch, const float* amax_a, const float* amax_b,
                                   void* amax_c, unsigned amax_epoch, resel_stream_t stream) {
    if (!fused_args_ok(A, lda, strideA, a_kcontig, B, ldb, strideB, b_kcontig, C, ldc, M, N, K, batch, amax_a, amax_b, amax_c, workspace)) return RESEL_EINVAL;
    if (!Y || ldy % 4 || strideY % 4 || ldy <= 0 || !aligned16(Y) || !a_kcontig || M < 256 || N % 128) return RESEL_EINVAL;
    hipStream_t s = (hipStream_t)stream;
    const int Mm = M / 256 * 256, tail = M - Mm, rows = 2 * (Mm / 256) + (tail ? 1 : 0);
    float* part = dbias ? (float*)workspace : nullptr;
    int rc = gemm_bf3_launch(A, lda, strideA, a_kcontig, B, ldb, strideB, b_kcontig, nullptr, 0, 4, C, ldc, strideC, nullptr, Mm, N, K, batch, 2,
                             s, amax_a, amax_b, (unsigned long long*)amax_c, amax_epoch, Y, ldy, strideY, part, rows);
    if (rc != RESEL_OK) return rc;
    if (tail) {
        char* ws2 = (char*)workspace + ((size_t)rows * N * batch * sizeof(float) + 255) / 256 * 256;
        rc = resel_gemm_f32x(A + (int64_t)Mm * lda, lda, strideA, 1, B, ldb, strideB, b_kcontig, nullptr, 0, 0, C + (int64_t)Mm * ldc, ldc, strideC, ws2,
                             tail, N, K, batch, 2, amax_a, amax_b, nullptr, 0u, stream);
        if (rc != RESEL_OK) return rc;
        hipLaunchKernelGGL(dact_tail_kernel, dim3((N + 63) / 64, batch), dim3(256), 0, s, C + (int64_t)Mm * ldc, ldc, strideC, Y + (int64_t)Mm * ldy, ldy, strideY,
                           tail, N, part ? part + (int64_t)(rows - 1) * N : nullptr, (int64_t)rows * N, AmaxOut{(unsigned long long*)amax_c, amax_epoch});
    }
    if (dbias) launch_colsum(part, N, rows, N, dbias, s, 1, 0, batch);
    return launch_status();
}

extern "C" int resel_gemm_f32_head(const float* A, int64_t lda, int64_t strideA, int a_kcontig,
                                   const float* B, int64_t ldb, int64_t strideB, int b_kcontig,
                                   const float* bias, int64_t strideBias, const float* w3, int64_t strideW3, const float* b3,
                                   float* C, int64_t ldc, int64_t strideC, float* q, void* workspace,
                                   int M, int N, int K, int batch, const float* amax_a, const float* amax_b,
                                   void* amax_c, unsigned amax_epoch, resel_stream_t stream) {
    if (!fused_args_ok(A, lda, strideA, a_kcontig, B, ldb, strideB, b_kcontig, C, ldc, M, N, K, batch, amax_a, amax_b, amax_c, workspace)) return RESEL_EINVAL;
    if (!w3 || !q || strideW3 % 4 || !aligned16(w3)) return RESEL_EINVAL;
    const int rc = gemm_bf3_launch(A, lda, strideA, a_kcontig, B, ldb, strideB, b_kcontig, bias, strideBias, 5, C, ldc, strideC, nullptr, M, N, K, batch, 2,
                                   (hipStream_t)stream, amax_a, amax_b, (unsigned long long*)amax_c, amax_epoch, w3, 0, strideW3, (float*)workspace);
    if (rc != RESEL_OK) return rc;
    hipLaunchKernelGGL(head_fold_kernel, dim3((M + 255) / 256, batch), dim3(256), 0, (hipStream_t)stream, (const float*)workspace,
                       2 * ((N + 127) / 128), M, b3, q);
    return launch_status();
}
```

recurrent-offpolicy-rl_amd/csrc/misc.hip:

```cpp
#include "resel_common.h"
#include <cstdint>

extern "C" int resel_abi_version(void) { return 9; }

namespace { const unsigned long long* g_drop_base = nullptr; }
namespace resel { const unsigned long long* dropout_offset_base() { return g_drop_base; } }
extern "C" int resel_dropout_offset_base(const void* base) {
    if (base && ((uintptr_t)base & 7)) return RESEL_EINVAL;
    g_drop_base = (const unsigned long long*)base;
    return RESEL_OK;
}
extern "C" const char* resel_build_info(void) { return "resel_hip gfx950 (CDNA4, wave64) built " __DATE__ " " __TIME__; }

#include <utility>
#include <vector>
namespace resel {
namespace {
bool g_prof_enabled = false;
std::vector<std::pair<hipEvent_t, hipEvent_t>> g_prof_ev[RESEL_PROF_NSLOTS];
}
bool prof_on() { return g_prof_enabled; }
void prof_push(int slot, hipEvent_t a, hipEvent_t b) {
    if (slot >= 0 && slot < RESEL_PROF_NSLOTS) g_prof_ev[slot].emplace_back(a, b);
}
}

extern "C" int resel_profile_enable(int on) {
    resel::g_prof_enabled = on != 0;
    return RESEL_OK;
}

extern "C" int resel_profile_collect(int kernel_id, double* total_us, int* launches) {
    if (kernel_id < 0 || kernel_id >= RESEL_PROF_NSLOTS || !total_us || !launches) return RESEL_EINVAL;
    double tot = 0.0;
    int n = 0;
    for (auto& pr : resel::g_prof_ev[kernel_id]) {
        float ms = 0.f;
        if (hipEventSynchronize(pr.second) == hipSuccess && hipEventElapsedTime(&ms, pr.first, pr.second) == hipSuccess) {
            tot += 1e3 * ms;
            ++n;
        }
        (void)hipEventDestroy(pr.first);
        (void)hipEventDestroy(pr.second);
    }
    resel::g_prof_ev[kernel_id].clear();
    *total_us = tot;
    *launches = n;
    return RESEL_OK;
}

namespace {
struct PlaceBlock { const float* src; long long ld; int r0, nr, c0, nc; };
struct PlaceArgs { PlaceBlock b[8]; int n; };
__global__ __launch_bounds__(256) void place_blocks_kernel(float* __restrict__ out, long long ld_out, long long total, int cols, PlaceArgs a) {
    const long long i = (long long)blockIdx.x * 256 + threadIdx.x;
    if (i >= total) return;
    const int r = (int)(i / cols), c = (int)(i - (long long)r * cols);
    float v = 0.f;
#pragma unroll
    for (int k = 0; k < 8; ++k) {
        if (k < a.n) {
            const int rr = r - a.b[k].r0, cc = c - a.b[k].c0;
            if ((unsigned)rr < (unsigned)a.b[k].nr && (unsigned)cc < (unsigned)a.b[k].nc) v = a.b[k].src[(long long)rr * a.b[k].ld + cc];
        }
    }
    out[(long long)r * ld_out + c] = v;
}
}

extern "C" int resel_place_blocks(float* out, int64_t ld_out, int rows, int cols, int nblk, const float* const* src, const int64_t* ld_src,
                                  const int* r0, const int* nr, const int* c0, const int* nc, resel_stream_t stream) {
    if (!out || rows <= 0 || cols <= 0 || ld_out < cols || nblk < 0 || nblk > 8 || (nblk && (!src || !ld_src || !r0 || !nr || !c0 || !nc))) return RESEL_EINVAL;
    PlaceArgs a{};
    a.n = nblk;
    for (int k = 0; k < nblk; ++k) {
        if (!src[k] || nr[k] <= 0 || nc[k] <= 0 || r0[k] < 0 || c0[k] < 0 || r0[k] + nr[k] > rows || c0[k] + nc[k] > cols || ld_src[k] < nc[k]) return RESEL_EINVAL;
        a.b[k] = PlaceBlock{src[k], (long long)ld_src[k], r0[k], nr[k], c0[k], nc[k]};
    }
    const long long total = (long long)rows * cols;
    hipLaunchKernelGGL(place_blocks_kernel, dim3((unsigned)((total + 255) / 256)), dim3(256), 0, (hipStream_t)stream, out, (long long)ld_out, total, cols, a);
    return resel::launch_status();
}
```

recurrent-offpolicy-rl_amd/offpolicy_rnn/hip/_lib.py:

```python
import ctypes
import os
from ctypes import c_float, c_int, c_int64, c_size_t, c_uint64, c_void_p

_HERE = os.path.dirname(os.path.abspath(__file__))
LIB_PATH = os.environ.get('RESEL_HIP_LIBRARY') or os.path.join(_HERE, 'libresel_hip.so')
ABI_VERSION = 9
_lib = None

P, I, L, F, S, U = c_void_p, c_int, c_int64, c_float, c_void_p, c_uint64
E = ctypes.c_uint

SIGNATURES = {
    'resel_abi_version': (c_int, []),
    'resel_build_info': (ctypes.c_char_p, []),
    'resel_profile_enable': (c_int, [I]),
    'resel_profile_collect': (c_int, [I, P, P]),
    'resel_selective_scan_ckpt_bytes': (c_size_t, [I, I, I, I]),
    'resel_selective_scan_fwd_workspace_bytes': (c_size_t, [I, I, I, I, I]),
    'resel_selective_scan_fwd': (c_int, [P, L, P, L, P, L, P, P, L, P, L, P, P, P, P, L, P, P, P, I, I, I, I, I, I, P, E, S]),
    'resel_selective_scan_bwd_workspace_bytes': (c_size_t, [I, I, I, I, I]),
    'resel_selective_scan_bwd': (c_int, [P, L, P, L, P, L, P, P, L, P, L, P, P, P, P, L, P,
                                         P, L, P, L, P, L, P, L, P, L, P, P, P, P, I, I, I, I, I, I, P, P, E, S]),
    'resel_causal_conv1d_fwd': (c_int, [P, L, P, P, P, P, L, I, I, I, I, I, P, E, S]),
    'resel_causal_conv1d_bwd_workspace_bytes': (c_size_t, [I, I, I, I]),
    'resel_causal_conv1d_bwd': (c_int, [P, L, P, P, P, P, L, P, L, P, P, P, I, I, I, I, I, P, E, S]),
    'resel_causal_conv1d_bwd2': (c_int, [P, L, P, P, P, P, L, P, L, P, L, P, P, P, I, I, I, I, I, P, E, S]),
    'resel_add_layernorm_fwd': (c_int, [P, P, P, P, P, P, P, I, I, F, I, I, P, E, S]),
    'resel_add_layernorm_bwd_workspace_bytes': (c_size_t, [I, I]),
    'resel_add_layernorm_bwd': (c_int, [P, P, P, P, P, P, P, P, P, P, I, I, I, I, I, P, E, S]),
    'resel_linrec_real_fwd': (c_int, [P, P, L, P, P, P, I, I, I, I, P, E, S]),
    'resel_linrec_real_bwd': (c_int, [P, P, L, P, P, P, P, P, P, L, I, I, I, I, P, E, S]),
    'resel_linrec_complex_fwd': (c_int, [P, P, L, P, P, P, P, P, P, P, P, I, I, I, P, E, S]),
    'resel_linrec_complex_bwd_workspace_bytes': (c_size_t, [I, I, I]),
    'resel_place_blocks': (c_int, [P, L, I, I, I, P, P, P, P, P, P, S]),
    'resel_lru_params_fwd': (c_int, [P, P, I, S]),
    'resel_lru_params_bwd': (c_int, [P, P, P, I, S]),
    'resel_linrec_complex_bwd': (c_int, [P, P, L, P, P, P, P, P, P, P, P, P, P, P, P, L, P, P, P, P, I, I, I, S]),
    'resel_gru_workspace_bytes': (c_size_t, [I, I, I]),
    'resel_gru_seq_fwd': (c_int, [P, P, P, P, P, P, P, I, I, I, S]),
    'resel_gru_seq_bwd': (c_int, [P, P, P, P, P, P, P, P, I, I, I, S]),
    'resel_gru_multi_workspace_bytes': (c_size_t, [I, I, I, I]),
    'resel_gru_multi_fwd': (c_int, [I, P, P, P, P, P, P, P, I, I, I, S]),
    'resel_gru_multi_form': (c_int, [I, I, I]),
    'resel_attn_varlen_fwd_workspace_bytes': (c_size_t, [I, I]),
    'resel_attn_varlen_fwd': (c_int, [P, P, P, P, P, P, I, I, I, I, I, F, F, U, U, S]),
    'resel_attn_varlen_bwd_workspace_bytes': (c_size_t, [I, I, I, I, I]),
    'resel_attn_varlen_bwd': (c_int, [P, P, P, P, P, P, P, P, I, I, I, I, I, F, F, U, U, S]),
    'resel_dropout': (c_int, [P, P, L, F, U, U, S]),
    'resel_dropout_offset_base': (c_int, [P]),
    'resel_gelu_dropout_fwd': (c_int, [P, P, L, F, U, U, P, E, S]),
    'resel_gelu_dropout_bwd': (c_int, [P, P, P, L, F, U, U, P, E, S]),
    'resel_tanh_gaussian_fwd': (c_int, [P, P, P, P, P, I, I, S]),
    'resel_tanh_gaussian_bwd': (c_int, [P, P, P, P, P, I, I, S]),
    'resel_sac_target': (c_int, [P, P, I, P, P, P, P, P, F, P, P, P, P, I, I, S]),
    'resel_sac_target_phase': (c_int, [I, P, P, I, P, P, P, P, P, F, P, P, P, P, P, I, I, S]),
    'resel_masked_loss_workspace_bytes': (c_size_t, []),
    'resel_q_loss_fwd': (c_int, [P, P, P, P, P, I, I, S]),
    'resel_q_loss_bwd': (c_int, [P, P, P, P, P, I, I, S]),
    'resel_actor_loss_fwd': (c_int, [P, P, P, P, P, P, I, I, I, I, S]),
    'resel_actor_loss_bwd': (c_int, [P, P, P, P, P, P, I, I, I, I, S]),
    'resel_sac_target_local': (c_int, [P, P, I, P, P, P, P, P, F, P, P, P, P, P, I, I, S]),
    'resel_guard_apply_slots': (c_int, [P, I, P, S]),
    'resel_sac_target_workspace_bytes': (c_size_t, [I]),
    'resel_soft_update': (c_int, [P, P, F, L, S]),
    'resel_adamw_flat': (c_int, [P, P, P, P, L, P, P, P, I, F, F, F, I, P, S]),
    'resel_adamw_flat_bc': (c_int, [P, P, P, P, L, P, P, P, I, F, F, F, F, F, P, S]),
    'resel_adamw_flat_dev': (c_int, [P, P, P, P, L, P, P, P, I, F, F, F, P, P, S]),
    'resel_sumsq_workspace_bytes': (c_size_t, [L]),
    'resel_sumsq': (c_int, [P, L, P, P, S]),
    'resel_bias_act_fwd': (c_int, [P, P, L, I, L, I, S]),
    'resel_bias_act_bwd_workspace_bytes': (c_size_t, [L, I, L]),
    'resel_bias_act_bwd': (c_int, [P, L, P, L, P, P, P, L, I, L, I, P, E, S]),
    'resel_ensemble_head_fwd': (c_int, [P, P, P, P, P, L, I, L, S]),
    'resel_ensemble_head_bwd_workspace_bytes': (c_size_t, [L, I, L]),
    'resel_ensemble_head_bwd': (c_int, [P, P, P, P, P, P, P, L, I, L, P, E, S]),
    'resel_gemm_f32_workspace_bytes': (c_size_t, [I, I, I, I]),
    'resel_gemm_f32': (c_int, [P, L, L, I, P, L, L, I, P, L, I, P, L, L, P, I, I, I, I, I, S]),
    'resel_gemm_f32x': (c_int, [P, L, L, I, P, L, L, I, P, L, I, P, L, L, P, I, I, I, I, I, P, P, P, E, S]),
    'resel_amax_segments': (c_int, [P, P, P, I, P, E, S]),
    'resel_amax_state_bytes': (c_size_t, []),
    'resel_amax': (c_int, [P, L, L, I, I, I, P, E, P, S]),
    'resel_gemm_f32_fused_supported': (c_int, [I, I, I, I, L, L]),
    'resel_gemm_f32_fused_workspace_bytes': (c_size_t, [I, I, I, I, I]),
    'resel_gemm_f32_dact': (c_int, [P, L, L, I, P, L, L, I, P, L, L, P, L, L, P, P, I, I, I, I, P, P, P, E, S]),
    'resel_gemm_f32_head': (c_int, [P, L, L, I, P, L, L, I, P, L, P, L, P, P, L, L, P, P, I, I, I, I, P, P, P, E, S]),
    'resel_amax_check': (c_int, [P, L, L, I, I, I, P, P, I, S]),
    'resel_gemm_bf16_workspace_bytes': (c_size_t, [I, I, I]),
    'resel_gemm_bf16': (c_int, [P, L, I, I, P, L, I, I, P, P, L, I, P, I, I, I, S]),
    'resel_colsum_bf16_workspace_bytes': (c_size_t, [I, I]),
    'resel_colsum_bf16': (c_int, [P, L, I, I, P, P, S]),
    'resel_gather_trajs': (c_int, [P, I, L, P, I, I, I, I, I, I, I, I, I, P, I, P, S]),
    'resel_mamba_conv_step': (c_int, [P, L, P, L, P, L, L, L, I, P, P, P, I, I, I, I, S]),
    'resel_selective_state_update': (c_int, [P, L, P, L, P, P, L, P, P, P, P, P, L, P, I, I, I, I, S]),
    'resel_atb_workspace_bytes': (c_size_t, [L, I, I]),
    'resel_atb': (c_int, [P, L, I, P, L, I, P, I, P, L, S]),
    'resel_attn_decode': (c_int, [P, L, P, P, I, P, P, F, I, I, I, I, S]),
}


class ReselHipUnavailable(RuntimeError):
    pass


def lib():
    global _lib
    if _lib is not None:
        return _lib
    if not os.path.exists(LIB_PATH):
        raise ReselHipUnavailable(
            f'RESeL-HIP: {LIB_PATH} not found. The MI355X kernels are the only implementation of the hot path; '
            f'build them with `python -c "import __graft_entry__ as g; g.build()"` (or `make -C recurrent-offpolicy-rl_amd/csrc`).')
    handle = ctypes.CDLL(LIB_PATH)
    for name, (res, args) in SIGNATURES.items():
        fn = getattr(handle, name, None)
        if fn is None:
            raise ReselHipUnavailable(f'RESeL-HIP: symbol {name} missing from {LIB_PATH} (stale build?)')
        fn.restype = res
        fn.argtypes = args
    if handle.resel_abi_version() != ABI_VERSION:
        raise ReselHipUnavailable(f'RESeL-HIP: ABI {handle.resel_abi_version()} != expected {ABI_VERSION}; rebuild the library')
    _lib = handle
    return _lib


def check(rc: int, what: str):
    if rc != 0:
        raise RuntimeError(f'RESeL-HIP: {what} failed with code {rc} '
                           f'({ {-1: "RESEL_EINVAL (shape/alignment/null)", -2: "RESEL_ELAUNCH"}.get(rc, "?")})')
```

recurrent-offpolicy-rl_amd/offpolicy_rnn/hip/ops.py:

```python
import ctypes
import os
from typing import Optional

import torch

from ._lib import check, lib


def _need_cuda(name, *ts):
    for t in ts:
        if t is not None and not t.is_cuda:
            raise RuntimeError(f'RESeL-HIP: {name} needs CUDA tensors (got a {t.device} tensor); the HIP kernels are the '
                               f'only implementation of this op - there is no CPU fallback.')


def _p(t: Optional[torch.Tensor]):
    return None if t is None else ctypes.c_void_p(t.data_ptr())


if hasattr(torch._C, '_cuda_getCurrentRawStream') and hasattr(torch._C, '_cuda_getDevice'):
    def _stream():
        return ctypes.c_void_p(torch._C._cuda_getCurrentRawStream(torch._C._cuda_getDevice()))
else:
    def _stream():
# ... 1219 lines not shown

GEMM_SPLIT = int(os.environ['RESEL_GEMM_SPLIT']) if os.environ.get('RESEL_GEMM_SPLIT') else None


def gemm_split():
    if GEMM_SPLIT is not None:
        return GEMM_SPLIT
    return 2 if torch.get_float32_matmul_precision() == 'highest' else 3



_GEMM_WS_BYTES = {}


AMAX_SLOTS = 2048
AMAX_WORDS = 128
AMAX_PREPASS_FRACTION = 0.16
_AMAX_ARENA = {}
_AMAX_EPOCH = [0]
LAST_AMAX = None
LAST_SPLIT = [None]


def publish_amax(slot):
    global LAST_AMAX
    LAST_AMAX = slot


def apply_tagged(fn, whole, *args):
    global LAST_AMAX
    LAST_AMAX = None
    out = fn(*args)
    tag_amax(out[0] if type(out) is tuple else out, LAST_AMAX, whole)
    LAST_AMAX = None
    return out


_AMAX_SERIAL = [0]
AMAX_GENERATION = [0]
_EPOCH_RESET_AT = 0x60000000
_STORES = None


def register_store(store):
    global _STORES
    if _STORES is None:
        import weakref
        _STORES = weakref.WeakSet()
    _STORES.add(store)


def amax_slot(device):
    _AMAX_SERIAL[0] += 1
    ar = _AMAX_ARENA.get(device)
    if ar is None:
        buf = torch.zeros(AMAX_SLOTS * AMAX_WORDS, dtype=torch.int64, device=device)
        ar = _AMAX_ARENA[device] = [buf, 0, list(buf.view(AMAX_SLOTS, AMAX_WORDS).unbind(0))]
    if _AMAX_EPOCH[0] >= _EPOCH_RESET_AT and not torch.cuda.is_current_stream_capturing():
        amax_maintenance(force=True)
    if _AMAX_EPOCH[0] >= 0x7ffffff0:
        raise RuntimeError('RESeL-HIP: magnitude epochs exhausted inside one captured region')
    _AMAX_EPOCH[0] += 1
    i = ar[1]
    ar[1] = (i + 1) % AMAX_SLOTS
    h = ar[2][i]
    h._resel_serial = _AMAX_SERIAL[0]
    return h, _AMAX_EPOCH[0]


def amax_maintenance(force=False):
    if not force and _AMAX_EPOCH[0] < _EPOCH_RESET_AT:
        return False
    _AMAX_EPOCH[0] = 0
    AMAX_GENERATION[0] += 1
    PARAM_EPOCH[0] += 1
    for ar in _AMAX_ARENA.values():
        torch.cuda.synchronize(ar[0].device)
        ar[0].zero_()
        for h in ar[2]:
            h._resel_serial = None
    for st in (list(_STORES) if _STORES is not None else []):
        st._amax = None
    return True


def amax_arena_zero(device):
    ar = _AMAX_ARENA.get(device)
    if ar is not None:
        ar[0].zero_()


def keep_handles(*hs):
    return tuple((h, getattr(h, '_resel_serial', None)) for h in hs)


def handle_alive(kept):
    h, serial = kept
    return h if h is not None and getattr(h, '_resel_serial', None) == serial else None


def live_handles(kept):
    return tuple(handle_alive(k) for k in kept)


def _taggable(t):
    return not (isinstance(t, torch.nn.Parameter) or (t.is_leaf and t.requires_grad))


def tag_amax(t, handle, whole=False):
    if t is not None:
        ok = handle is not None and _taggable(t)
        serial = getattr(handle, '_resel_serial', None) if ok else None
        t._resel_amax = (handle, t._version, serial) if ok else None
        base = getattr(t, '_base', None)
        if whole and base is not None:
            base._resel_amax = (handle, base._version, serial) if (ok and _taggable(base)) else None
    return t


def amax_of(t):
    for obj in (t, getattr(t, '_base', None)):
        if obj is not None:
            tg = getattr(obj, '_resel_amax', None)
            if tg is not None and tg[1] == obj._version and getattr(tg[0], '_resel_serial', None) == tg[2]:
                return tg[0]
    return None


AMAX_VERIFY = os.environ.get('RESEL_AMAX_VERIFY', '0') == '1'
_VERIFY_ERR = {}
_VERIFY_CALLS = []
_VERIFY_TAG = [0]


class AmaxBoundError(RuntimeError):
    pass


@torch.no_grad()
def amax_check(x, handle, what=''):
    assert x.dtype == torch.float32 and x.stride(-1) == 1 and x.dim() in (2, 3)
    err = _VERIFY_ERR.get(x.device)
    if err is None:
        err = _VERIFY_ERR[x.device] = torch.zeros(4, dtype=torch.int32, device=x.device)
    _VERIFY_TAG[0] += 1
    _VERIFY_CALLS.append((_VERIFY_TAG[0], f'{what} {tuple(x.shape)} strides {tuple(x.stride())}'))
    del _VERIFY_CALLS[:-4096]
    batch = x.shape[0] if x.dim() == 3 else 1
    check(lib().resel_amax_check(_p(x), x.stride(-2), x.stride(0) if x.dim() == 3 and batch > 1 else 0, x.shape[-2], x.shape[-1], batch,
                                 _p(handle), _p(err), _VERIFY_TAG[0], _stream()), 'amax_check')


def amax_verify_raise(device=None):
    for dev, err in list(_VERIFY_ERR.items()):
        if device is not None:
            d = torch.device(device)
            if d.type != dev.type or (d.index is not None and d.index != dev.index):
                continue
        e = err.cpu()
        if int(e[0]) == 0:
            continue
        err.zero_()
        tag = int(e[2])
        what = dict(_VERIFY_CALLS).get(tag, '?')
        got = float(e[1:2].view(torch.float32)[0])
        bound = float(e[3:4].view(torch.float32)[0])
        raise AmaxBoundError(f'RESeL-HIP: GEMM mode 2 was given a magnitude handle BELOW its operand: max |x| = {got:.6g} > bound {bound:.6g} '
                             f'(first report: check #{tag}: {what}; {int(e[0])} reporting waves) - the fp16 planes would overflow to inf')


@torch.no_grad()
def amax(x):
    _need_cuda('amax', x)
    assert x.dtype == torch.float32 and x.stride(-1) == 1 and x.dim() in (2, 3)
    out, epoch = amax_slot(x.device)
    batch = x.shape[0] if x.dim() == 3 else 1
    check(lib().resel_amax(_p(x), x.stride(-2), x.stride(0) if x.dim() == 3 and batch > 1 else 0, x.shape[-2], x.shape[-1], batch,
                           _p(out), epoch, None, _stream()), 'amax')
    return out


def amax_value(handle):
    w = handle.view(torch.int64).cpu()[::16][:8]
    ep = (w >> 32) & 0xffffffff
    lo = (w[ep == ep.max()] & 0xffffffff).to(torch.int32)
    return float(lo.view(torch.float32).max())


PARAM_EPOCH = [0]


@torch.no_grad()
def amax_segments(flat, begin, length, handles):
    _need_cuda('amax_segments', flat, begin, length, handles)
    _AMAX_EPOCH[0] += 1
    check(lib().resel_amax_segments(_p(flat), _p(begin), _p(length), int(begin.numel()), _p(handles), _AMAX_EPOCH[0], _stream()), 'amax_segments')


def weight_amax(p):
    ref = getattr(p, '_resel_store', None)
    if ref is None or not amax_tracking():
        return None
    return ref[0].amax_handle(ref[1], p)


def _slot_args(want, device):
    if not want:
        return None, None, 0
    slot, epoch = amax_slot(device)
    return slot, _p(slot), epoch


def amax_tracking():
    return gemm_split() == 2


def _operand_handles(A, B, amax_a, amax_b):
    ha = amax_a if amax_a is not None else amax_of(A)
    hb = amax_b if amax_b is not None else amax_of(B)
    return weight_amax(A) if ha is None else ha, weight_amax(B) if hb is None else hb


def _prepass(x):
    h = amax(x)
    tag_amax(x, h)
    return h


def _verify_operands(A, B, ha, hb, what):
    amax_check(A, ha, 'A of ' + what)
    amax_check(B, hb, 'B of ' + what)


def _gemm_done(out, slot, split):
    LAST_SPLIT[0] = split
    return tag_amax(out, slot)


@torch.no_grad()
def gemm_f32(A, B, a_kcontig=True, b_kcontig=True, bias=None, act=None, out=None, split=None, amax_a=None, amax_b=None, amax_out=None):
    _need_cuda('gemm_f32', A, B)
    batched = A.dim() == 3
    assert A.stride(-1) == 1 and B.stride(-1) == 1 and A.dtype == torch.float32 and B.dtype == torch.float32
    sa_, sb_ = A.shape, B.shape
    batch = sa_[0] if batched else 1
    M, K = (sa_[-2], sa_[-1]) if a_kcontig else (sa_[-1], sa_[-2])
    N = sb_[-2] if b_kcontig else sb_[-1]
    assert (sb_[-1] if b_kcontig else sb_[-2]) == K and (not batched or sb_[0] == batch)
    if out is None:
        out = torch.empty((batch, M, N) if batched else (M, N), dtype=torch.float32, device=A.device)
    assert out.stride(-1) == 1
    GEMM_FLOPS[0] += 2.0 * M * N * K * batch
    L = lib()
    key = (M, N, K, batch)
    nb = _GEMM_WS_BYTES.get(key)
    if nb is None:
        nb = _GEMM_WS_BYTES[key] = L.resel_gemm_f32_workspace_bytes(M, N, K, batch)
    ws = _ws(nb, A.device) if nb else None
    bs = 0
    if bias is not None:
        bias = bias.reshape(batch, N) if batched else bias.reshape(N)
        bs = bias.stride(0) if batched else 0
    multi = batch > 1
    split = gemm_split() if split is None else int(split)
    ha = hb = None
    if split == 2:
        if K < 32 or M <= 128:
            split = 6
        else:
            ha, hb = _operand_handles(A, B, amax_a, amax_b)
            if ha is None or hb is None:
                t_gemm = 2.0 * M * N * K * batch / 1.5e8
                cost = (0.0 if ha is not None else 4.0 * M * K * batch / 4.5e6 + 2.5) + (0.0 if hb is not None else 4.0 * N * K * batch / 4.5e6 + 2.5)
                if cost <= AMAX_PREPASS_FRACTION * t_gemm:
                    ha = _prepass(A) if ha is None else ha
                    hb = _prepass(B) if hb is None else hb
                else:
                    split = 6
    if AMAX_VERIFY and split == 2:
        _verify_operands(A, B, ha, hb, f'gemm M={M} N={N} K={K} batch={batch}')
    slot, slot_p, epoch = amax_out if amax_out is not None else \
        _slot_args(amax_tracking() and act != GEMM_ACCUMULATE and M * N * batch >= (1 << 20), A.device)
    check(L.resel_gemm_f32x(_p(A), A.stride(-2), A.stride(0) if multi else 0, int(a_kcontig), _p(B), B.stride(-2),
                            B.stride(0) if multi else 0, int(b_kcontig), _p(bias), bs, 2 if act == GEMM_ACCUMULATE else 3 if act == GEMM_SOFTPLUS else ACT_IDS[act], _p(out), out.stride(-2),
                            out.stride(0) if multi else 0, _p(ws), M, N, K, batch, split, _p(ha) if split == 2 else None,
                            _p(hb) if split == 2 else None, slot_p, epoch, _stream()), 'gemm_f32')
    publish_amax(slot)
    return _gemm_done(out, slot, split)


def _forced_handles(A, B, amax_a, amax_b):
    ha, hb = _operand_handles(A, B, amax_a, amax_b)
    return _prepass(A) if ha is None else ha, _prepass(B) if hb is None else hb


def gemm_fused_ok(kind, M, N, K, *mats):
    if os.environ.get('RESEL_GEMM_FUSED', '1') == '0' or gemm_split() != 2 or not gemm_f32_ok(*mats) or not rows_aligned16(*mats):
        return False
    ld = max(int(t.stride(-2)) for t in mats)
    return bool(lib().resel_gemm_f32_fused_supported(int(kind), int(M), int(N), int(K), ld, ld))


@torch.no_grad()
def gemm_f32_dact(A, B, b_kcontig, Y, out, need_dbias=True, amax_a=None, amax_b=None):
    _need_cuda('gemm_f32_dact', A, B, Y, out)
    batched = A.dim() == 3
    batch = A.shape[0] if batched else 1
    M, K = A.shape[-2], A.shape[-1]
    N = B.shape[-2] if b_kcontig else B.shape[-1]
    assert (B.shape[-1] if b_kcontig else B.shape[-2]) == K and Y.shape[-2:] == (M, N) and out.shape[-2:] == (M, N)
    assert A.stride(-1) == 1 and B.stride(-1) == 1 and Y.stride(-1) == 1 and out.stride(-1) == 1
    ha, hb = _forced_handles(A, B, amax_a, amax_b)
    if AMAX_VERIFY:
        _verify_operands(A, B, ha, hb, f'gemm_dact M={M} N={N} K={K} batch={batch}')
    GEMM_FLOPS[0] += 2.0 * M * N * K * batch
    L = lib()
    ws = _ws(L.resel_gemm_f32_fused_workspace_bytes(M, N, K, batch, 4), A.device)
    dbias = torch.empty(batch, N, dtype=torch.float32, device=A.device) if need_dbias else None
    multi = batched and batch > 1
    slot, slot_p, epoch = _slot_args(amax_tracking() and M * N * batch >= (1 << 20), A.device)
    check(L.resel_gemm_f32_dact(_p(A), A.stride(-2), A.stride(0) if multi else 0, 1, _p(B), B.stride(-2), B.stride(0) if multi else 0, int(b_kcontig),
                                _p(Y), Y.stride(-2), Y.stride(0) if multi else 0, _p(out), out.stride(-2), out.stride(0) if multi else 0,
                                _p(dbias), _p(ws), M, N, K, batch, _p(ha), _p(hb), slot_p, epoch, _stream()), 'gemm_f32_dact')
    return _gemm_done(out, slot, 2), dbias


@torch.no_grad()
def gemm_f32_head(A, B, b_kcontig, bias, w3, b3, amax_a=None, amax_b=None):
    _need_cuda('gemm_f32_head', A, B, bias, w3)
    batch, M, K = A.shape
    N = B.shape[-2] if b_kcontig else B.shape[-1]
    assert A.stride(-1) == 1 and B.stride(-1) == 1 and w3.shape == (batch, N) and w3.is_contiguous() and bias.shape == (batch, N) and bias.stride(-1) == 1
    ha, hb = _forced_handles(A, B, amax_a, amax_b)
    if AMAX_VERIFY:
        _verify_operands(A, B, ha, hb, f'gemm_head M={M} N={N} K={K} batch={batch}')
    GEMM_FLOPS[0] += 2.0 * M * N * K * batch
    L = lib()
    ws = _ws(L.resel_gemm_f32_fused_workspace_bytes(M, N, K, batch, 5), A.device)
    a = torch.empty(batch, M, N, dtype=torch.float32, device=A.device)
    q = torch.empty(batch, M, dtype=torch.float32, device=A.device)
    multi = batch > 1
    slot, slot_p, epoch = _slot_args(amax_tracking() and M * N * batch >= (1 << 20), A.device)
    check(L.resel_gemm_f32_head(_p(A), A.stride(-2), A.stride(0) if multi else 0, 1, _p(B), B.stride(-2), B.stride(0) if multi else 0, int(b_kcontig),
                                _p(bias), bias.stride(0) if multi else 0, _p(w3), N, _p(b3), _p(a), a.stride(-2), a.stride(0) if multi else 0, _p(q), _p(ws),
                                M, N, K, batch, _p(ha), _p(hb), slot_p, epoch, _stream()), 'gemm_f32_head')
    return _gemm_done(a, slot, 2), q


@torch.no_grad()
def conv_step(x, window, weight, bias, d_conv, layout, act):
    _need_cuda('conv_step', x, window)
    B, Di, K = x.shape[0], x.shape[1], d_conv
    W, sd, sk = (K, K, 1) if layout == 'dk' else (K - 1, 1, Di)
    assert window.shape == (B, Di * W) and window.stride(1) == 1 and x.stride(1) == 1
    new = torch.empty((B, Di * W), dtype=torch.float32, device=x.device)
    xc = torch.empty((B, Di), dtype=torch.float32, device=x.device)
    check(lib().resel_mamba_conv_step(_p(x), x.stride(0), _p(window), window.stride(0), _p(new), new.stride(0), sd, sk, W,
                                      _p(weight), _p(bias), _p(xc), B, Di, K, int(bool(act)), _stream()), 'mamba_conv_step')
    return xc, new


@torch.no_grad()
def selective_state_update(state, xc, x_db, dt_w, dt_b, A_log, D, z=None):
    _need_cuda('selective_state_update', state, xc, x_db)
    B, Di = xc.shape
    R = dt_w.shape[1]
    N = (x_db.shape[1] - R) // 2
    assert state.shape == (B, Di * N) and state.stride(1) == 1 and x_db.stride(1) == 1 and xc.is_contiguous()
    new = torch.empty((B, Di * N), dtype=torch.float32, device=xc.device)
    y = torch.empty_like(xc)
    check(lib().resel_selective_state_update(_p(state), state.stride(0), _p(new), new.stride(0), _p(xc), _p(x_db), x_db.stride(0),
                                             _p(dt_w), _p(dt_b), _p(A_log), _p(D), _p(z), 0 if z is None else z.stride(0), _p(y),
                                             B, Di, N, R, _stream()), 'selective_state_update')
    return y, new


@torch.no_grad()
def mamba_step(hidden, xz, conv_w, conv_b, xproj_w, dt_w, dt_b, A_log, D, d_conv, d_state):
    Di, K = xz.shape[1] // 2, d_conv
    xc, window = conv_step(xz[:, :Di], hidden[:, :Di * K], conv_w, conv_b, K, 'dk', True)
    x_db = gemm_f32(xc, xproj_w, True, True)
    y, state = selective_state_update(hidden[:, Di * K:], xc, x_db, dt_w, dt_b, A_log, D, xz[:, Di:])
    return y, torch.cat((window, state), dim=-1)


@torch.no_grad()
def attn_decode(qkv, kv_cache, pos, slopes, scale):
    _need_cuda('attn_decode', qkv, kv_cache)
    B, _, H, hd = qkv.shape
    assert qkv.dtype == torch.bfloat16 and kv_cache.dtype == torch.bfloat16 and qkv.is_contiguous() and kv_cache.is_contiguous()
    assert kv_cache.shape[0] >= B and kv_cache.shape[2:] == (2, H, hd)
    out = torch.empty((B, H, hd), dtype=torch.bfloat16, device=qkv.device)
    dev = pos if torch.is_tensor(pos) else None
    check(lib().resel_attn_decode(_p(qkv), 3 * H * hd, _p(kv_cache), _p(dev), 0 if dev is not None else int(pos), _p(slopes), _p(out),
                                  float(scale), B, H, hd, kv_cache.shape[1], _stream()), 'attn_decode')
    return out


@torch.no_grad()
def soft_update_(target_flat, online_flat, tau):
    _need_cuda('soft_update', target_flat, online_flat)
    PARAM_EPOCH[0] += 1
    check(lib().resel_soft_update(_p(target_flat), _p(online_flat), float(tau), target_flat.numel(), _stream()), 'soft_update')


def adamw_bias_corrections(beta1, beta2, step):
    t = float(step)
    return 1.0 - beta1 ** t, (1.0 - beta2 ** t) ** 0.5


@torch.no_grad()
def adamw_flat_(p, g, m, v, seg_end, seg_lr, seg_wd, step, beta1=0.9, beta2=0.999, eps=1e-8, grad_scale=None):
    _need_cuda('adamw_flat', p, g, m, v, seg_end, seg_lr, seg_wd)
    PARAM_EPOCH[0] += 1
    bc1, bc2_sqrt = adamw_bias_corrections(beta1, beta2, step)
    check(lib().resel_adamw_flat_bc(_p(p), _p(g), _p(m), _p(v), p.numel(), _p(seg_end), _p(seg_lr), _p(seg_wd), int(seg_end.numel()),
                                    float(beta1), float(beta2), float(eps), bc1, bc2_sqrt, _p(grad_scale), _stream()), 'adamw_flat')


@torch.no_grad()
def adamw_flat_dev_(p, g, m, v, seg_end, seg_lr, seg_wd, bias_corrections, beta1=0.9, beta2=0.999, eps=1e-8, grad_scale=None):
    _need_cuda('adamw_flat_dev', p, g, m, v, seg_end, seg_lr, seg_wd, bias_corrections)
    PARAM_EPOCH[0] += 1
    check(lib().resel_adamw_flat_dev(_p(p), _p(g), _p(m), _p(v), p.numel(), _p(seg_end), _p(seg_lr), _p(seg_wd), int(seg_end.numel()),
                                     float(beta1), float(beta2), float(eps), _p(bias_corrections), _p(grad_scale), _stream()), 'adamw_flat_dev')


@torch.no_grad()
def sumsq(x, out=None):
    _need_cuda('sumsq', x)
    out = torch.empty(1, dtype=torch.float32, device=x.device) if out is None else out
    ws = _ws(lib().resel_sumsq_workspace_bytes(x.numel()), x.device)
    check(lib().resel_sumsq(_p(x), x.numel(), _p(out), _p(ws), _stream()), 'sumsq')
    return out
```

recurrent-offpolicy-rl_amd/offpolicy_rnn/models/ensemble_linear_model.py:

```python
import torch
import torch.nn as nn

from ..hip import ops


def _unit(t):
    return t if t.stride(-1) == 1 else t.contiguous()


class _SharedInput(torch.autograd.Function):

    @staticmethod
    def forward(ctx, x2, weight, bias, act, x_part=None, col0=0, ax=None):
        E, n_in, n_out = weight.shape
        w_cat = weight.permute(1, 0, 2).reshape(n_in, E * n_out)
        x2 = x2 if x2.stride(-1) == 1 else x2.contiguous()
        y2 = ops.gemm_f32(x2, w_cat, True, False, None if bias is None else bias.reshape(E * n_out), act, amax_a=ax,
                          amax_b=ops.weight_amax(weight))
        ax = ax if ax is not None else ops.amax_of(x2)
        ctx.save_for_backward(x2, w_cat, y2 if act is not None else None)
        ctx.ax = ops.keep_handles(ax)[0]
        ctx.dims = (E, n_in, n_out, bias is not None, act)
        ctx.part = None if x_part is None else (col0, x_part.shape[-1], tuple(x_part.shape))
        return y2.view(-1, E, n_out).transpose(0, 1)

    @staticmethod
    def backward(ctx, g):
        x2, w_cat, y2 = ctx.saved_tensors
        E, n_in, n_out, has_bias, act = ctx.dims
        g2 = g.transpose(0, 1).reshape(-1, E * n_out)
        need_db = has_bias and ctx.needs_input_grad[2]
        if act is not None:
            g2, db = ops.bias_act_bwd(g2, y2, g2.shape[0], act, need_db)
        else:
            db = g2.sum(dim=0, keepdim=True) if need_db else None
        g2 = g2 if g2.stride(-1) == 1 else g2.contiguous()
        dx = None
        if ctx.needs_input_grad[0]:
            dx = ops.gemm_f32(g2, w_cat, True, True)
        dw = None
        if ctx.needs_input_grad[1]:
            dw = ops.gemm_f32(x2, g2, False, False, amax_a=ops.handle_alive(ctx.ax))
            dw = dw.view(n_in, E, n_out).permute(1, 0, 2)
        dpart = None
        if ctx.part is not None and ctx.needs_input_grad[4]:
            col0, k, shape = ctx.part
            wp = w_cat[col0:col0 + k]
            dpart = ops.gemm_f32(g2, wp, True, True).view(shape)
        return dx, dw, None if db is None else db.view(E, 1, n_out), None, dpart, None, None


def _member_wgrad(x3, gy, ax=None):
    return ops.gemm_f32(_unit(x3), _unit(gy), False, False, amax_a=ax)


def _member_dgrad(gy, weight, like):
    E, M, _ = gy.shape
    n_in = weight.shape[1]
    if like.stride(0) < like.stride(1):
        dx = torch.empty(M, E, n_in, dtype=gy.dtype, device=gy.device).transpose(0, 1)
    else:
        dx = torch.empty(E, M, n_in, dtype=gy.dtype, device=gy.device)
    return ops.gemm_f32(_unit(gy), weight, True, True, out=dx)


class _PerMember(torch.autograd.Function):
    @staticmethod
    def forward(ctx, x3, weight, bias, act, ax=None):
        E, M, _ = x3.shape
        x3 = _unit(x3)
        y = ops.gemm_f32(x3, weight, True, False, bias, act, amax_a=ax)
        ax = ax if ax is not None else ops.amax_of(x3)
        ctx.save_for_backward(x3, weight, y if act is not None else None)
        ctx.ax = ops.keep_handles(ax)[0]
        ctx.cfg = (bias is not None, act)
        return y

    @staticmethod
    def backward(ctx, g):
        x3, weight, y = ctx.saved_tensors
        has_bias, act = ctx.cfg
        E, M, n_out = g.shape
        need_db = has_bias and ctx.needs_input_grad[2]
        if act is not None or (need_db and n_out % 4 == 0):
            gy, db = ops.bias_act_bwd(g.reshape(E * M, n_out), None if y is None else y.view(E * M, n_out), M, act, need_db)
            gy = gy.view(E, M, n_out)
            db = None if db is None else db.view(E, 1, n_out)
        else:
            gy, db = g, (g.sum(dim=1, keepdim=True) if need_db else None)
        dx = _member_dgrad(gy, weight, x3) if ctx.needs_input_grad[0] else None
        dw = _member_wgrad(x3, gy, ops.handle_alive(ctx.ax)) if ctx.needs_input_grad[1] else None
        return dx, dw, db, None, None


class _Head(torch.autograd.Function):

    @staticmethod
    def forward(ctx, x3, w2, b2, w3, b3, ax=None):
        E, M, _ = x3.shape
        H = w2.shape[2]
        x3 = _unit(x3)
        a = ops.gemm_f32(x3, w2, True, False, amax_a=ax)
        ax = ax if ax is not None else ops.amax_of(x3)
        ctx.ax = ops.keep_handles(ax)[0]
        w3v = w3.reshape(E, H)
        q = ops.ensemble_head_fwd_(a, b2.reshape(E, H), w3v, None if b3 is None else b3.reshape(E))
        ctx.save_for_backward(x3, w2, w3v, a)
        ctx.has_b3 = b3 is not None
        return q.view(E, M, 1)

    @staticmethod
    def backward(ctx, gq):
        x3, w2, w3v, a = ctx.saved_tensors
        E, M, H = a.shape
        gq2 = gq.reshape(E, M)
        gy, db2, dw3 = ops.ensemble_head_bwd(gq2, a, w3v)
        dx = _member_dgrad(gy, w2, x3) if ctx.needs_input_grad[0] else None
        dw2 = _member_wgrad(x3, gy, ops.handle_alive(ctx.ax))
        db3 = gq2.sum(dim=1).view(E, 1, 1) if ctx.has_b3 else None
        return dx, dw2, db2.view(E, 1, H), dw3.view(E, H, 1), db3, None


class _CriticMLP(torch.autograd.Function):

    @staticmethod
    def forward(ctx, x2, W1, b1, W2, b2, W3, b3, x_part, col0, ax):
        E, n_in, H1 = W1.shape
        H2 = W2.shape[2]
        M = x2.shape[0]
        w_cat = W1.permute(1, 0, 2).reshape(n_in, E * H1)
        y2 = ops.gemm_f32(x2, w_cat, True, False, b1.reshape(E * H1), 'elu', amax_a=ax, amax_b=ops.weight_amax(W1))
        h_x = ax if ax is not None else ops.amax_of(x2)
        h_a1 = ops.amax_of(y2)
        a1 = y2.view(M, E, H1).transpose(0, 1)
        w3v = W3.reshape(E, H2)
        a2, q = ops.gemm_f32_head(a1, W2, False, b2.reshape(E, H2), w3v, None if b3 is None else b3.reshape(E), amax_a=h_a1,
                                  amax_b=ops.weight_amax(W2))
        ctx.save_for_backward(x2, w_cat, y2, W2, w3v, a2)
        ctx.handles = ops.keep_handles(h_x, h_a1)
        ctx.dims = (E, n_in, H1, H2, M, b3 is not None)
        ctx.part = None if x_part is None else (col0, x_part.shape[-1], tuple(x_part.shape))
        return q.view(E, M, 1)

    @staticmethod
    def backward(ctx, gq):
        x2, w_cat, y2, W2, w3v, a2 = ctx.saved_tensors
        E, n_in, H1, H2, M, has_b3 = ctx.dims
        h_x, h_a1 = ops.live_handles(ctx.handles)
        need = ctx.needs_input_grad
        gq2 = gq.reshape(E, M)
        gy2, db2, dw3 = ops.ensemble_head_bwd(gq2, a2, w3v)
        a1 = y2.view(M, E, H1).transpose(0, 1)
        dw2 = _member_wgrad(a1, gy2, h_a1) if need[3] else None
        db3 = gq2.sum(dim=1).view(E, 1, 1) if (has_b3 and need[6]) else None
        g1 = torch.empty(M, E, H1, dtype=torch.float32, device=x2.device).transpose(0, 1)
        _, db1 = ops.gemm_f32_dact(gy2, W2, True, a1, g1, need_dbias=bool(need[2]), amax_b=ops.weight_amax(W2))
        g2 = g1.transpose(0, 1).reshape(M, E * H1)
        ops.tag_amax(g2, ops.amax_of(g1))
        dx = ops.gemm_f32(g2, w_cat, True, True) if need[0] else None
        dw1 = None
        if need[1]:
            dw1 = ops.gemm_f32(x2, g2, False, False, amax_a=h_x).view(n_in, E, H1).permute(1, 0, 2)
        dpart = None
        if ctx.part is not None and need[7]:
            col0, k, shape = ctx.part
            dpart = ops.gemm_f32(g2, w_cat[col0:col0 + k], True, True).view(shape)
        return (dx, dw1, None if db1 is None else db1.view(E, 1, H1), dw2, db2.view(E, 1, H2) if need[4] else None,
                dw3.view(E, H2, 1) if need[5] else None, db3, dpart, None, None)


def critic_mlp_fusable(l0, act0, l1, act1, l2, act2, x) -> bool:
    if not (isinstance(l0, EnsembleLinear) and isinstance(l1, EnsembleLinear) and isinstance(l2, EnsembleLinear)):
        return False
    elu = lambda a: isinstance(a, nn.ELU) and a.alpha == 1.0
    if not (elu(act0) and elu(act1) and isinstance(act2, nn.Identity) and l0.use_bias and l1.use_bias):
        return False
    E = l0.active_members()
    if l1.active_members() != E or l2.active_members() != E or x.dtype != torch.float32 or not x.is_cuda:
        return False
    n_in, H1 = l0.weight.shape[1:]
    H2 = l1.weight.shape[2]
    if l1.weight.shape[1] != H1 or l2.weight.shape[1] != H2 or l2.weight.shape[2] != 1 or x.shape[-1] != n_in:
        return False
    nd = x.dim()
    if nd >= 5 or (nd in (3, 4) and (l0.desire_ndim is None or l0.desire_ndim == nd) and x.shape[0] == E):
        return False
    if not all(l.desire_ndim is None or l.desire_ndim == nd + 1 for l in (l1, l2)):
        return False
    M = x.numel() // n_in
    x2 = x.reshape(-1, n_in)
    return (min(n_in, H1, H2) >= 32 and H1 % 32 == 0 and H2 % 32 == 0 and ops.gemm_f32_ok(x2) and ops.rows_aligned16(x2)
            and ops.gemm_fused_ok(5, M, H2, H1, l1.weight) and ops.gemm_fused_ok(4, M, H1, H2, l1.weight))


def critic_mlp(l0: 'EnsembleLinear', l1: 'EnsembleLinear', l2: 'EnsembleLinear', x: torch.Tensor, grad_part=None) -> torch.Tensor:
    W1, b1 = l0.active_params()
    W2, b2 = l1.active_params()
    W3, b3 = l2.active_params()
    E, n_in, _ = W1.shape
    lead = tuple(x.shape[:-1])
    ax = ops.amax_of(x)
    if grad_part is not None:
        q = _CriticMLP.apply(x.detach().reshape(-1, n_in), W1, b1, W2, b2, W3, b3, grad_part[0], grad_part[1], ax)
    else:
        q = _CriticMLP.apply(x.reshape(-1, n_in), W1, b1, W2, b2, W3, b3, None, 0, ax)
    return q.reshape((E,) + lead + (1,))


def ensemble_head(hidden: 'EnsembleLinear', out: 'EnsembleLinear', x: torch.Tensor) -> torch.Tensor:
    w2, b2 = hidden.active_params()
    w3, b3 = out.active_params()
    E, n_in, H = w2.shape
    lead = tuple(x.shape[1:-1])
    q = _Head.apply(x.reshape(E, -1, n_in), w2, b2, w3, b3, ops.amax_of(x))
    return q.reshape((E,) + lead + (1,))


def head_fusable(hidden, hidden_act, out, out_act, x) -> bool:
    return (isinstance(hidden, EnsembleLinear) and isinstance(out, EnsembleLinear) and isinstance(hidden_act, nn.ELU)
            and hidden_act.alpha == 1.0 and isinstance(out_act, nn.Identity) and hidden.use_bias
            and out.weight.shape[2] == 1 and out.weight.shape[1] == hidden.weight.shape[2] and hidden.weight.shape[2] % 4 == 0
            and x.dim() >= 3 and x.shape[0] == hidden.active_members() and x.dtype == torch.float32
            and (hidden.desire_ndim is None or hidden.desire_ndim == x.dim()))


class EnsembleLinear(nn.Module):
    def __init__(self, input_dim: int, output_dim: int, num_ensemble: int, bias: bool = True, desire_ndim: int = None):
        super().__init__()
        self.use_bias = bias
        self.desire_ndim = desire_ndim
        self.num_ensemble = num_ensemble
        self.weight = nn.Parameter(torch.zeros(num_ensemble, input_dim, output_dim))
        if bias:
            self.bias = nn.Parameter(torch.zeros(num_ensemble, 1, output_dim))
        nn.init.trunc_normal_(self.weight, std=1 / (2 * input_dim ** 0.5))
        self.member_index = None

    def active_members(self) -> int:
        return self.num_ensemble if self.member_index is None else int(self.member_index.numel())

    def active_params(self):
        b = self.bias if self.use_bias else None
        if self.member_index is None:
            return self.weight, b
        return self.weight.index_select(0, self.member_index), None if b is None else b.index_select(0, self.member_index)

    def forward(self, x: torch.Tensor, act: str = None, grad_part=None) -> torch.Tensor:
        W, b = self.active_params()
        E, n_in, n_out = W.shape
        nd = x.dim()
        shared = True
        if nd == 3:
            shared = not ((self.desire_ndim is None or self.desire_ndim == 3) and x.shape[0] == E)
        elif nd == 4:
            shared = not ((self.desire_ndim is None or self.desire_ndim == 4) and x.shape[0] == E)
        elif nd == 5:
            shared = False
        ax = ops.amax_of(x)
        if shared:
            lead = tuple(x.shape[:-1])
            if grad_part is not None:
                y = ops.apply_tagged(_SharedInput.apply, True, x.detach().reshape(-1, n_in), W, b, act, grad_part[0], grad_part[1], ax)
            else:
                y = ops.apply_tagged(_SharedInput.apply, True, x.reshape(-1, n_in), W, b, act, None, 0, ax)
        else:
            assert grad_part is None, 'grad_part is a shared-input feature'
            lead = tuple(x.shape[1:-1])
            y = ops.apply_tagged(_PerMember.apply, True, x.reshape(E, -1, n_in), W, b, act, ax)
        return y.reshape((E,) + lead + (n_out,))
```

Before: 3.087 million env-steps/s.

## Skip head activation stores when critic gradients are only needed for inputs

Adds store forms to the fused critic head GEMM. With no grad it skips writing the hidden activation entirely. When only input gradients are needed (actor update through frozen critic) it stores w3*ELU'(pre) instead. The backward then folds the per-row dq scale into the dact GEMM epilogue, skipping the separate head-backward and weight-gradient work. This cuts memory traffic and kernel launches at the cost of more epilogue branching and new scale paths in the dact kernel and tail kernel.

```diff
diff --git a/include/resel_hip.h b/include/resel_hip.h
--- a/include/resel_hip.h
+++ b/include/resel_hip.h
@@ -189,12 +189,24 @@
                         float* C, int64_t ldc, int64_t strideC, float* dbias, void* workspace,
                         int M, int N, int K, int batch, const float* amax_a, const float* amax_b,
                         void* amax_c, unsigned amax_epoch, resel_stream_t stream);
+int resel_gemm_f32_dact_rs(const float* A, int64_t lda, int64_t strideA, int a_kcontig,
+                           const float* B, int64_t ldb, int64_t strideB, int b_kcontig,
+                           const float* Y, int64_t ldy, int64_t strideY, const float* rs,
+                           float* C, int64_t ldc, int64_t strideC, float* dbias, void* workspace,
+                           int M, int N, int K, int batch, const float* amax_a, const float* amax_b,
+                           void* amax_c, unsigned amax_epoch, resel_stream_t stream);
 int resel_gemm_f32_head(const float* A, int64_t lda, int64_t strideA, int a_kcontig,
                         const float* B, int64_t ldb, int64_t strideB, int b_kcontig,
                         const float* bias, int64_t strideBias, const float* w3, int64_t strideW3, const float* b3,
                         float* C, int64_t ldc, int64_t strideC, float* q, void* workspace,
                         int M, int N, int K, int batch, const float* amax_a, const float* amax_b,
                         void* amax_c, unsigned amax_epoch, resel_stream_t stream);
+int resel_gemm_f32_head_form(const float* A, int64_t lda, int64_t strideA, int a_kcontig,
+                             const float* B, int64_t ldb, int64_t strideB, int b_kcontig,
+                             const float* bias, int64_t strideBias, const float* w3, int64_t strideW3, const float* b3,
+                             float* C, int64_t ldc, int64_t strideC, int form, float* q, void* workspace,
+                             int M, int N, int K, int batch, const float* amax_a, const float* amax_b,
+                             void* amax_c, unsigned amax_epoch, resel_stream_t stream);
 int resel_place_blocks(float* out, int64_t ld_out, int rows, int cols, int nblk, const float* const* src, const int64_t* ld_src,
                        const int* r0, const int* nr, const int* c0, const int* nc, resel_stream_t stream);
 
diff --git a/recurrent-offpolicy-rl_amd/csrc/gemm_bf3.hip b/recurrent-offpolicy-rl_amd/csrc/gemm_bf3.hip
--- a/recurrent-offpolicy-rl_amd/csrc/gemm_bf3.hip
+++ b/recurrent-offpolicy-rl_amd/csrc/gemm_bf3.hip
@@ -29,6 +29,9 @@
     int64_t ldaux, sAux;
     float* red;
     int redrows;
+    const float* rs;
+    int64_t sRs;
+    int form;
 };
 
 __device__ __forceinline__ int plane_off(int row, int c) {
@@ -971,14 +974,26 @@
                 mul(std::integral_constant<int, 0>{}); mul(std::integral_constant<int, 1>{}); mul(std::integral_constant<int, 2>{});
                 mul(std::integral_constant<int, 3>{}); mul(std::integral_constant<int, 4>{}); mul(std::integral_constant<int, 5>{});
                 mul(std::integral_constant<int, 6>{}); mul(std::integral_constant<int, 7>{});
-                if (p.red) {
-#pragma unroll
-                    for (int b = 0; b < 2; ++b) {
-                        const float c = cs[b] + __shfl_xor(cs[b], 32, 64);
-                        if (lh == 0) p.red[((int64_t)cur.z * p.redrows + 2 * (cur.m0 / BM) + (w >> 1)) * p.N + cur.n0 + wn + 32 * b + li] = c;
-                    }
-                }
-                amax_publish_wave(cmx, p.amaxC);
+                auto finish = [&]() {
+                    if (p.red) {
+#pragma unroll
+                        for (int b = 0; b < 2; ++b) {
+                            const float c = cs[b] + __shfl_xor(cs[b], 32, 64);
+                            if (lh == 0) p.red[((int64_t)cur.z * p.redrows + 2 * (cur.m0 / BM) + (w >> 1)) * p.N + cur.n0 + wn + 32 * b + li] = c;
+                        }
+                    }
+                    amax_publish_wave(cmx, p.amaxC);
+                };
+                const bool scaled = p.rs != nullptr;
+                float* rsl = reinterpret_cast<float*>(lds + 3 * PLA + 2 * PLB) + 128 * w;
+                if (scaled) {
+                    const float* rp = p.rs + (int64_t)cur.z * p.sRs + cur.m0 + wm + lane;
+                    const float r0 = rp[0], r1 = rp[64];
+                    rsl[lane] = r0; rsl[lane + 64] = r1;
+                    cs[0] = cs[1] = cmx = 0.f;
+                } else {
+                    finish();
+                }
 #pragma unroll
                 for (int b = 0; b < 2; ++b) {
 #pragma unroll
@@ -988,12 +1003,23 @@
                         float* q = C + (int64_t)(cur.m0 + wm + 32 * a + (lane >> 3)) * p.ldc + cur.n0 + wn + 32 * b + 4 * (lane & 7);
 #pragma unroll
                         for (int g = 0; g < 4; ++g) {
-                            const float4 t = rdp[g * 8 * 10];
+                            float4 t = rdp[g * 8 * 10];
+                            if (scaled) {
+                                const float r = rsl[32 * a + 8 * g + (lane >> 3)];
+                                t.x *= r; t.y *= r; t.z *= r; t.w *= r;
+                                cmx = amax4(cmx, t);
+                                if (p.red) rdp[g * 8 * 10] = t;
+                            }
                             typedef float f4v __attribute__((ext_vector_type(4)));
                             __builtin_nontemporal_store(f4v{t.x, t.y, t.z, t.w}, reinterpret_cast<f4v*>(q + (int64_t)(8 * g) * p.ldc));
                         }
-                    }
-                }
+                        if (scaled && p.red) {
+#pragma unroll
+                            for (int e = 0; e < 16; ++e) cs[b] += wr[((e & 3) + 8 * (e >> 2)) * 40];
+                        }
+                    }
+                }
+                if (scaled) finish();
                 continue;
             }
             if (full_m && cur.n0 + BN <= p.N && act != 2) {
@@ -1012,7 +1038,7 @@
 #pragma unroll
                         for (int e = 0; e < 16; ++e) v[e] = softplus_nb(v[e]);
                     }
-                    if (p.amaxC.slot && !DACT) {
+                    if (p.amaxC.slot && !DACT && !(HEAD && p.form)) {
 #pragma unroll
                         for (int e = 0; e < 16; e += 2) cmax = fmaxf(cmax, fmaxf(__builtin_fabsf(v[e]), __builtin_fabsf(v[e + 1])));
                     }
@@ -1029,6 +1055,12 @@
                             if (p.amaxC.slot) cmax = amax4(cmax, t);
                         }
                         if (HEAD) qr[g] += (t.x * w3.x + t.y * w3.y) + (t.z * w3.z + t.w * w3.w);
+                        if (HEAD && p.form) {
+                            if (p.form == 2) continue;
+                            t.x = w3.x * (t.x > 0.f ? 1.f : t.x + 1.f); t.y = w3.y * (t.y > 0.f ? 1.f : t.y + 1.f);
+                            t.z = w3.z * (t.z > 0.f ? 1.f : t.z + 1.f); t.w = w3.w * (t.w > 0.f ? 1.f : t.w + 1.f);
+                            if (p.amaxC.slot) cmax = amax4(cmax, t);
+                        }
                         if (p.ntst) {
                             typedef float f4v __attribute__((ext_vector_type(4)));
                             __builtin_nontemporal_store(f4v{t.x, t.y, t.z, t.w}, reinterpret_cast<f4v*>(q + (int64_t)(8 * g) * p.ldc));
@@ -1109,6 +1141,11 @@
                         const float w3 = p.aux[(int64_t)cur.z * p.sAux + n];
 #pragma unroll
                         for (int e = 0; e < 16; ++e) qe[e] += v[e] * w3;
+                        if (p.form == 2) continue;
+                        if (p.form == 1) {
+#pragma unroll
+                            for (int e = 0; e < 16; ++e) v[e] = w3 * (v[e] > 0.f ? 1.f : v[e] + 1.f);
+                        }
                     }
                     float* crow = C + (int64_t)mb * p.ldc + n;
                     if (act == 2) {
@@ -1193,19 +1230,21 @@
 int gemm_bf3_launch(const float* A, int64_t lda, int64_t strideA, int a_kcontig, const float* B, int64_t ldb, int64_t strideB, int b_kcontig,
                     const float* bias, int64_t strideBias, int act, float* C, int64_t ldc, int64_t strideC, void* workspace,
                     int M, int N, int K, int batch, int split, hipStream_t s, const float* amaxA, const float* amaxB,
-                    unsigned long long* amax_c, unsigned amax_epoch, const float* aux, int64_t ldaux, int64_t strideAux, float* red, int redrows) {
+                    unsigned long long* amax_c, unsigned amax_epoch, const float* aux, int64_t ldaux, int64_t strideAux, float* red, int redrows,
+                    const float* rs, int64_t strideRs, int form) {
     if (split == 2 && (!amaxA || !amaxB)) return RESEL_EINVAL;
     Plan pl = make_plan<BM, BN, GRID>(M, N, K, batch);
     if (act >= 4) {
         if (split != 2 || !gemm_bf3_fused_ok(M, N, K, lda, ldb) || !aux) return RESEL_EINVAL;
         if (act == 4 && (M % BM || N % BN)) return RESEL_EINVAL;
+        if (form < 0 || form > 2) return RESEL_EINVAL;
         const long nbt = (long)((M + BM - 1) / BM) * ((N + BN - 1) / BN) * batch;
         pl = Plan{(int)nbt, 0, 1, (K + BK - 1) / BK * BK};
     }
     if (pl.nsplit && (!workspace || !aligned16(workspace))) return RESEL_EINVAL;
     Params p{A, B, bias, C, (float*)workspace, lda, ldb, ldc, strideA, strideB, strideC, strideBias, M, N, K, act,
              (M + BM - 1) / BM, (N + BN - 1) / BN, pl.nfull, pl.nsplit, pl.nsl, pl.kslice, amaxA, amaxB, AmaxOut{amax_c, amax_epoch}, g_nt,
-             aux, ldaux, strideAux, red, redrows};
+             aux, ldaux, strideAux, red, redrows, act == 4 ? rs : nullptr, strideRs, act == 5 ? form : 0};
     const int64_t total = (int64_t)pl.nfull + (int64_t)pl.nsplit * pl.nsl;
     dim3 grid((unsigned)std::min<int64_t>(total, GRID));
     int rc;
diff --git a/recurrent-offpolicy-rl_amd/csrc/gemm_f32.hip b/recurrent-offpolicy-rl_amd/csrc/gemm_f32.hip
--- a/recurrent-offpolicy-rl_amd/csrc/gemm_f32.hip
+++ b/recurrent-offpolicy-rl_amd/csrc/gemm_f32.hip
@@ -6,7 +6,7 @@
                     const float* bias, int64_t strideBias, int act, float* C, int64_t ldc, int64_t strideC, void* workspace,
                     int M, int N, int K, int batch, int split, hipStream_t s, const float* amaxA, const float* amaxB,
                     unsigned long long* amax_c, unsigned amax_epoch, const float* aux = nullptr, int64_t ldaux = 0, int64_t strideAux = 0,
-                    float* red = nullptr, int redrows = 0);
+                    float* red = nullptr, int redrows = 0, const float* rs = nullptr, int64_t strideRs = 0, int form = 0);
 bool gemm_bf3_fused_ok(int M, int N, int K, int64_t lda, int64_t ldb);
 }
 
@@ -532,7 +532,8 @@
 
 namespace {
 __global__ __launch_bounds__(256) void dact_tail_kernel(float* __restrict__ C, int64_t ldc, int64_t sC, const float* __restrict__ Y, int64_t ldy, int64_t sY,
-                                                        int rows, int N, float* __restrict__ part, int64_t part_stride, AmaxOut amax) {
+                                                        int rows, int N, float* __restrict__ part, int64_t part_stride, AmaxOut amax,
+                                                        const float* __restrict__ rs, int64_t sRs) {
     __shared__ float s_sum[4][64];
     const int c = blockIdx.x * 64 + (threadIdx.x & 63), rg = threadIdx.x >> 6, z = blockIdx.y;
     float acc = 0.f, mx = 0.f;
@@ -541,7 +542,8 @@
         const float* Yz = Y + (int64_t)z * sY + c;
         for (int r = rg; r < rows; r += 4) {
             const float y = Yz[(int64_t)r * ldy];
-            const float v = Cz[(int64_t)r * ldc] * (y > 0.f ? 1.f : y + 1.f);
+            float v = Cz[(int64_t)r * ldc] * (y > 0.f ? 1.f : y + 1.f);
+            if (rs) v *= rs[(int64_t)z * sRs + r];
             Cz[(int64_t)r * ldc] = v;
             acc += v;
             mx = fmaxf(mx, __builtin_fabsf(v));
@@ -554,19 +556,19 @@
 }
 }
 
-extern "C" int resel_gemm_f32_dact(const float* A, int64_t lda, int64_t strideA, int a_kcontig,
-                                   const float* B, int64_t ldb, int64_t strideB, int b_kcontig,
-                                   const float* Y, int64_t ldy, int64_t strideY,
-                                   float* C, int64_t ldc, int64_t strideC, float* dbias, void* workspace,
-                                   int M, int N, int K, int batch, const float* amax_a, const float* amax_b,
-                                   void* amax_c, unsigned amax_epoch, resel_stream_t stream) {
+extern "C" int resel_gemm_f32_dact_rs(const float* A, int64_t lda, int64_t strideA, int a_kcontig,
+                                      const float* B, int64_t ldb, int64_t strideB, int b_kcontig,
+                                      const float* Y, int64_t ldy, int64_t strideY, const float* rs,
+                                      float* C, int64_t ldc, int64_t strideC, float* dbias, void* workspace,
+                                      int M, int N, int K, int batch, const float* amax_a, const float* amax_b,
+                                      void* amax_c, unsigned amax_epoch, resel_stream_t stream) {
     if (!fused_args_ok(A, lda, strideA, a_kcontig, B, ldb, strideB, b_kcontig, C, ldc, M, N, K, batch, amax_a, amax_b, amax_c, workspace)) return RESEL_EINVAL;
     if (!Y || ldy % 4 || strideY % 4 || ldy <= 0 || !aligned16(Y) || !a_kcontig || M < 256 || N % 128) return RESEL_EINVAL;
     hipStream_t s = (hipStream_t)stream;
     const int Mm = M / 256 * 256, tail = M - Mm, rows = 2 * (Mm / 256) + (tail ? 1 : 0);
     float* part = dbias ? (float*)workspace : nullptr;
     int rc = gemm_bf3_launch(A, lda, strideA, a_kcontig, B, ldb, strideB, b_kcontig, nullptr, 0, 4, C, ldc, strideC, nullptr, Mm, N, K, batch, 2,
-                             s, amax_a, amax_b, (unsigned long long*)amax_c, amax_epoch, Y, ldy, strideY, part, rows);
+                             s, amax_a, amax_b, (unsigned long long*)amax_c, amax_epoch, Y, ldy, strideY, part, rows, rs, M, 0);
     if (rc != RESEL_OK) return rc;
     if (tail) {
         char* ws2 = (char*)workspace + ((size_t)rows * N * batch * sizeof(float) + 255) / 256 * 256;
@@ -574,9 +576,39 @@
                              tail, N, K, batch, 2, amax_a, amax_b, nullptr, 0u, stream);
         if (rc != RESEL_OK) return rc;
         hipLaunchKernelGGL(dact_tail_kernel, dim3((N + 63) / 64, batch), dim3(256), 0, s, C + (int64_t)Mm * ldc, ldc, strideC, Y + (int64_t)Mm * ldy, ldy, strideY,
-                           tail, N, part ? part + (int64_t)(rows - 1) * N : nullptr, (int64_t)rows * N, AmaxOut{(unsigned long long*)amax_c, amax_epoch});
+                           tail, N, part ? part + (int64_t)(rows - 1) * N : nullptr, (int64_t)rows * N, AmaxOut{(unsigned long long*)amax_c, amax_epoch},
+                           rs ? rs + Mm : nullptr, (int64_t)M);
     }
     if (dbias) launch_colsum(part, N, rows, N, dbias, s, 1, 0, batch);
+    return launch_status();
+}
+
+extern "C" int resel_gemm_f32_dact(const float* A, int64_t lda, int64_t strideA, int a_kcontig,
+                                   const float* B, int64_t ldb, int64_t strideB, int b_kcontig,
+                                   const float* Y, int64_t ldy, int64_t strideY,
+                                   float* C, int64_t ldc, int64_t strideC, float* dbias, void* workspace,
+                                   int M, int N, int K, int batch, const float* amax_a, const float* amax_b,
+                                   void* amax_c, unsigned amax_epoch, resel_stream_t stream) {
+    return resel_gemm_f32_dact_rs(A, lda, strideA, a_kcontig, B, ldb, strideB, b_kcontig, Y, ldy, strideY, nullptr, C, ldc, strideC, dbias, workspace,
+                                  M, N, K, batch, amax_a, amax_b, amax_c, amax_epoch, stream);
+}
+
+extern "C" int resel_gemm_f32_head_form(const float* A, int64_t lda, int64_t strideA, int a_kcontig,
+                                        const float* B, int64_t ldb, int64_t strideB, int b_kcontig,
+                                        const float* bias, int64_t strideBias, const float* w3, int64_t strideW3, const float* b3,
+                                        float* C, int64_t ldc, int64_t strideC, int form, float* q, void* workspace,
+                                        int M, int N, int K, int batch, const float* amax_a, const float* amax_b,
+                                        void* amax_c, unsigned amax_epoch, resel_stream_t stream) {
+    if (form < 0 || form > 2) return RESEL_EINVAL;
+    if (form == 2) { C = nullptr; ldc = 4; strideC = 0; amax_c = nullptr; }
+    if (!fused_args_ok(A, lda, strideA, a_kcontig, B, ldb, strideB, b_kcontig, form == 2 ? A : C, ldc, M, N, K, batch, amax_a, amax_b, amax_c, workspace)) return RESEL_EINVAL;
+    if (!w3 || !q || strideW3 % 4 || !aligned16(w3)) return RESEL_EINVAL;
+    const int rc = gemm_bf3_launch(A, lda, strideA, a_kcontig, B, ldb, strideB, b_kcontig, bias, strideBias, 5, C, ldc, strideC, nullptr, M, N, K, batch, 2,
+                                   (hipStream_t)stream, amax_a, amax_b, (unsigned long long*)amax_c, amax_epoch, w3, 0, strideW3, (float*)workspace, 0,
+                                   nullptr, 0, form);
+    if (rc != RESEL_OK) return rc;
+    hipLaunchKernelGGL(head_fold_kernel, dim3((M + 255) / 256, batch), dim3(256), 0, (hipStream_t)stream, (const float*)workspace,
+                       2 * ((N + 127) / 128), M, b3, q);
     return launch_status();
 }
 
@@ -586,12 +618,6 @@
                                    float* C, int64_t ldc, int64_t strideC, float* q, void* workspace,
                                    int M, int N, int K, int batch, const float* amax_a, const float* amax_b,
                                    void* amax_c, unsigned amax_epoch, resel_stream_t stream) {
-    if (!fused_args_ok(A, lda, strideA, a_kcontig, B, ldb, strideB, b_kcontig, C, ldc, M, N, K, batch, amax_a, amax_b, amax_c, workspace)) return RESEL_EINVAL;
-    if (!w3 || !q || strideW3 % 4 || !aligned16(w3)) return RESEL_EINVAL;
-    const int rc = gemm_bf3_launch(A, lda, strideA, a_kcontig, B, ldb, strideB, b_kcontig, bias, strideBias, 5, C, ldc, strideC, nullptr, M, N, K, batch, 2,
-                                   (hipStream_t)stream, amax_a, amax_b, (unsigned long long*)amax_c, amax_epoch, w3, 0, strideW3, (float*)workspace);
-    if (rc != RESEL_OK) return rc;
-    hipLaunchKernelGGL(head_fold_kernel, dim3((M + 255) / 256, batch), dim3(256), 0, (hipStream_t)stream, (const float*)workspace,
-                       2 * ((N + 127) / 128), M, b3, q);
-    return launch_status();
-}
+    return resel_gemm_f32_head_form(A, lda, strideA, a_kcontig, B, ldb, strideB, b_kcontig, bias, strideBias, w3, strideW3, b3, C, ldc, strideC, 0, q, workspace,
+                                    M, N, K, batch, amax_a, amax_b, amax_c, amax_epoch, stream);
+}
diff --git a/recurrent-offpolicy-rl_amd/csrc/misc.hip b/recurrent-offpolicy-rl_amd/csrc/misc.hip
--- a/recurrent-offpolicy-rl_amd/csrc/misc.hip
+++ b/recurrent-offpolicy-rl_amd/csrc/misc.hip
@@ -1,7 +1,7 @@
 #include "resel_common.h"
 #include <cstdint>
 
-extern "C" int resel_abi_version(void) { return 9; }
+extern "C" int resel_abi_version(void) { return 10; }
 
 namespace { const unsigned long long* g_drop_base = nullptr; }
 namespace resel { const unsigned long long* dropout_offset_base() { return g_drop_base; } }
diff --git a/recurrent-offpolicy-rl_amd/offpolicy_rnn/hip/_lib.py b/recurrent-offpolicy-rl_amd/offpolicy_rnn/hip/_lib.py
--- a/recurrent-offpolicy-rl_amd/offpolicy_rnn/hip/_lib.py
+++ b/recurrent-offpolicy-rl_amd/offpolicy_rnn/hip/_lib.py
@@ -4,7 +4,7 @@
 
 _HERE = os.path.dirname(os.path.abspath(__file__))
 LIB_PATH = os.environ.get('RESEL_HIP_LIBRARY') or os.path.join(_HERE, 'libresel_hip.so')
-ABI_VERSION = 9
+ABI_VERSION = 10
 _lib = None
 
 P, I, L, F, S, U = c_void_p, c_int, c_int64, c_float, c_void_p, c_uint64
@@ -84,6 +84,8 @@
     'resel_gemm_f32_fused_workspace_bytes': (c_size_t, [I, I, I, I, I]),
     'resel_gemm_f32_dact': (c_int, [P, L, L, I, P, L, L, I, P, L, L, P, L, L, P, P, I, I, I, I, P, P, P, E, S]),
     'resel_gemm_f32_head': (c_int, [P, L, L, I, P, L, L, I, P, L, P, L, P, P, L, L, P, P, I, I, I, I, P, P, P, E, S]),
+    'resel_gemm_f32_dact_rs': (c_int, [P, L, L, I, P, L, L, I, P, L, L, P, P, L, L, P, P, I, I, I, I, P, P, P, E, S]),
+    'resel_gemm_f32_head_form': (c_int, [P, L, L, I, P, L, L, I, P, L, P, L, P, P, L, L, I, P, P, I, I, I, I, P, P, P, E, S]),
     'resel_amax_check': (c_int, [P, L, L, I, I, I, P, P, I, S]),
     'resel_gemm_bf16_workspace_bytes': (c_size_t, [I, I, I]),
     'resel_gemm_bf16': (c_int, [P, L, I, I, P, L, I, I, P, P, L, I, P, I, I, I, S]),
diff --git a/recurrent-offpolicy-rl_amd/offpolicy_rnn/hip/ops.py b/recurrent-offpolicy-rl_amd/offpolicy_rnn/hip/ops.py
--- a/recurrent-offpolicy-rl_amd/offpolicy_rnn/hip/ops.py
+++ b/recurrent-offpolicy-rl_amd/offpolicy_rnn/hip/ops.py
@@ -1545,7 +1545,7 @@
 
 
 @torch.no_grad()
-def gemm_f32_dact(A, B, b_kcontig, Y, out, need_dbias=True, amax_a=None, amax_b=None):
+def gemm_f32_dact(A, B, b_kcontig, Y, out, need_dbias=True, amax_a=None, amax_b=None, rs=None):
     _need_cuda('gemm_f32_dact', A, B, Y, out)
     batched = A.dim() == 3
     batch = A.shape[0] if batched else 1
@@ -1553,6 +1553,7 @@
     N = B.shape[-2] if b_kcontig else B.shape[-1]
     assert (B.shape[-1] if b_kcontig else B.shape[-2]) == K and Y.shape[-2:] == (M, N) and out.shape[-2:] == (M, N)
     assert A.stride(-1) == 1 and B.stride(-1) == 1 and Y.stride(-1) == 1 and out.stride(-1) == 1
+    assert rs is None or (rs.is_cuda and rs.dtype == torch.float32 and rs.is_contiguous() and rs.numel() == batch * M)
     ha, hb = _forced_handles(A, B, amax_a, amax_b)
     if AMAX_VERIFY:
         _verify_operands(A, B, ha, hb, f'gemm_dact M={M} N={N} K={K} batch={batch}')
@@ -1562,14 +1563,17 @@
     dbias = torch.empty(batch, N, dtype=torch.float32, device=A.device) if need_dbias else None
     multi = batched and batch > 1
     slot, slot_p, epoch = _slot_args(amax_tracking() and M * N * batch >= (1 << 20), A.device)
-    check(L.resel_gemm_f32_dact(_p(A), A.stride(-2), A.stride(0) if multi else 0, 1, _p(B), B.stride(-2), B.stride(0) if multi else 0, int(b_kcontig),
-                                _p(Y), Y.stride(-2), Y.stride(0) if multi else 0, _p(out), out.stride(-2), out.stride(0) if multi else 0,
-                                _p(dbias), _p(ws), M, N, K, batch, _p(ha), _p(hb), slot_p, epoch, _stream()), 'gemm_f32_dact')
+    check(L.resel_gemm_f32_dact_rs(_p(A), A.stride(-2), A.stride(0) if multi else 0, 1, _p(B), B.stride(-2), B.stride(0) if multi else 0, int(b_kcontig),
+                                   _p(Y), Y.stride(-2), Y.stride(0) if multi else 0, _p(rs), _p(out), out.stride(-2), out.stride(0) if multi else 0,
+                                   _p(dbias), _p(ws), M, N, K, batch, _p(ha), _p(hb), slot_p, epoch, _stream()), 'gemm_f32_dact')
     return _gemm_done(out, slot, 2), dbias
 
 
-@torch.no_grad()
-def gemm_f32_head(A, B, b_kcontig, bias, w3, b3, amax_a=None, amax_b=None):
+HEAD_STORE_A, HEAD_STORE_U, HEAD_STORE_NONE = 0, 1, 2
+
+
+@torch.no_grad()
+def gemm_f32_head(A, B, b_kcontig, bias, w3, b3, amax_a=None, amax_b=None, form=HEAD_STORE_A):
     _need_cuda('gemm_f32_head', A, B, bias, w3)
     batch, M, K = A.shape
     N = B.shape[-2] if b_kcontig else B.shape[-1]
@@ -1580,13 +1584,14 @@
     GEMM_FLOPS[0] += 2.0 * M * N * K * batch
     L = lib()
     ws = _ws(L.resel_gemm_f32_fused_workspace_bytes(M, N, K, batch, 5), A.device)
-    a = torch.empty(batch, M, N, dtype=torch.float32, device=A.device)
+    assert form in (HEAD_STORE_A, HEAD_STORE_U, HEAD_STORE_NONE)
+    a = torch.empty(batch, M, N, dtype=torch.float32, device=A.device) if form != HEAD_STORE_NONE else None
     q = torch.empty(batch, M, dtype=torch.float32, device=A.device)
     multi = batch > 1
-    slot, slot_p, epoch = _slot_args(amax_tracking() and M * N * batch >= (1 << 20), A.device)
-    check(L.resel_gemm_f32_head(_p(A), A.stride(-2), A.stride(0) if multi else 0, 1, _p(B), B.stride(-2), B.stride(0) if multi else 0, int(b_kcontig),
-                                _p(bias), bias.stride(0) if multi else 0, _p(w3), N, _p(b3), _p(a), a.stride(-2), a.stride(0) if multi else 0, _p(q), _p(ws),
-                                M, N, K, batch, _p(ha), _p(hb), slot_p, epoch, _stream()), 'gemm_f32_head')
+    slot, slot_p, epoch = _slot_args(a is not None and amax_tracking() and M * N * batch >= (1 << 20), A.device)
+    check(L.resel_gemm_f32_head_form(_p(A), A.stride(-2), A.stride(0) if multi else 0, 1, _p(B), B.stride(-2), B.stride(0) if multi else 0, int(b_kcontig),
+                                     _p(bias), bias.stride(0) if multi else 0, _p(w3), N, _p(b3), _p(a), N, M * N if multi else 0, int(form), _p(q), _p(ws),
+                                     M, N, K, batch, _p(ha), _p(hb), slot_p, epoch, _stream()), 'gemm_f32_head')
     return _gemm_done(a, slot, 2), q
 
 
diff --git a/recurrent-offpolicy-rl_amd/offpolicy_rnn/models/ensemble_linear_model.py b/recurrent-offpolicy-rl_amd/offpolicy_rnn/models/ensemble_linear_model.py
--- a/recurrent-offpolicy-rl_amd/offpolicy_rnn/models/ensemble_linear_model.py
+++ b/recurrent-offpolicy-rl_amd/offpolicy_rnn/models/ensemble_linear_model.py
@@ -124,7 +124,7 @@
 class _CriticMLP(torch.autograd.Function):
 
     @staticmethod
-    def forward(ctx, x2, W1, b1, W2, b2, W3, b3, x_part, col0, ax):
+    def run_forward(x2, W1, b1, W2, b2, W3, b3, ax, form):
         E, n_in, H1 = W1.shape
         H2 = W2.shape[2]
         M = x2.shape[0]
@@ -135,26 +135,44 @@
         a1 = y2.view(M, E, H1).transpose(0, 1)
         w3v = W3.reshape(E, H2)
         a2, q = ops.gemm_f32_head(a1, W2, False, b2.reshape(E, H2), w3v, None if b3 is None else b3.reshape(E), amax_a=h_a1,
-                                  amax_b=ops.weight_amax(W2))
-        ctx.save_for_backward(x2, w_cat, y2, W2, w3v, a2)
-        ctx.handles = ops.keep_handles(h_x, h_a1)
+                                  amax_b=ops.weight_amax(W2), form=form)
+        return q.view(E, M, 1), (x2, w_cat, y2, W2, w3v, a2), (h_x, h_a1)
+
+    @staticmethod
+    def forward(ctx, x2, W1, b1, W2, b2, W3, b3, x_part, col0, ax):
+        E, n_in, H1 = W1.shape
+        H2 = W2.shape[2]
+        M = x2.shape[0]
+        need = ctx.needs_input_grad
+        form = ops.HEAD_STORE_NONE if not any(need) else ops.HEAD_STORE_U if not any(need[1:7]) else ops.HEAD_STORE_A
+        q, saved, (h_x, h_a1) = _CriticMLP.run_forward(x2, W1, b1, W2, b2, W3, b3, ax, form)
+        ctx.form = form
+        if form == ops.HEAD_STORE_NONE:
+            return q
+        ctx.save_for_backward(*saved)
+        a2 = saved[5]
+        ctx.handles = ops.keep_handles(h_x, h_a1, ops.amax_of(a2))
         ctx.dims = (E, n_in, H1, H2, M, b3 is not None)
         ctx.part = None if x_part is None else (col0, x_part.shape[-1], tuple(x_part.shape))
-        return q.view(E, M, 1)
+        return q
 
     @staticmethod
     def backward(ctx, gq):
         x2, w_cat, y2, W2, w3v, a2 = ctx.saved_tensors
         E, n_in, H1, H2, M, has_b3 = ctx.dims
-        h_x, h_a1 = ops.live_handles(ctx.handles)
+        h_x, h_a1, h_u2 = ops.live_handles(ctx.handles)
         need = ctx.needs_input_grad
         gq2 = gq.reshape(E, M)
-        gy2, db2, dw3 = ops.ensemble_head_bwd(gq2, a2, w3v)
         a1 = y2.view(M, E, H1).transpose(0, 1)
-        dw2 = _member_wgrad(a1, gy2, h_a1) if need[3] else None
-        db3 = gq2.sum(dim=1).view(E, 1, 1) if (has_b3 and need[6]) else None
         g1 = torch.empty(M, E, H1, dtype=torch.float32, device=x2.device).transpose(0, 1)
-        _, db1 = ops.gemm_f32_dact(gy2, W2, True, a1, g1, need_dbias=bool(need[2]), amax_b=ops.weight_amax(W2))
+        if ctx.form == ops.HEAD_STORE_U:
+            db2 = dw3 = dw2 = db3 = db1 = None
+            ops.gemm_f32_dact(a2, W2, True, a1, g1, need_dbias=False, amax_a=h_u2, amax_b=ops.weight_amax(W2), rs=gq2.contiguous())
+        else:
+            gy2, db2, dw3 = ops.ensemble_head_bwd(gq2, a2, w3v)
+            dw2 = _member_wgrad(a1, gy2, h_a1) if need[3] else None
+            db3 = gq2.sum(dim=1).view(E, 1, 1) if (has_b3 and need[6]) else None
+            _, db1 = ops.gemm_f32_dact(gy2, W2, True, a1, g1, need_dbias=bool(need[2]), amax_b=ops.weight_amax(W2))
         g2 = g1.transpose(0, 1).reshape(M, E * H1)
         ops.tag_amax(g2, ops.amax_of(g1))
         dx = ops.gemm_f32(g2, w_cat, True, True) if need[0] else None
@@ -200,7 +218,10 @@
     E, n_in, _ = W1.shape
     lead = tuple(x.shape[:-1])
     ax = ops.amax_of(x)
-    if grad_part is not None:
+    if not torch.is_grad_enabled():
+        with torch.no_grad():
+            q = _CriticMLP.run_forward(x.reshape(-1, n_in), W1, b1, W2, b2, W3, b3, ax, ops.HEAD_STORE_NONE)[0]
+    elif grad_part is not None:
         q = _CriticMLP.apply(x.detach().reshape(-1, n_in), W1, b1, W2, b2, W3, b3, grad_part[0], grad_part[1], ax)
     else:
         q = _CriticMLP.apply(x.reshape(-1, n_in), W1, b1, W2, b2, W3, b3, None, 0, ax)
```

After: 3.102 million env-steps/s, median of 6. No clear change (+0.5%).
